# mbed92/soft-grip

Hardware: AMD Instinct MI355X
Metric: env steps/sec (whole node) at batch=4096 (higher is better)
Workload: dtype f64; 1 GPU; configs[2]: 4096 envs/GPU, softbox scene (nv=118), stiffness ~ U(300,1400), reference 200-step squeeze schedule from reset, 7 substeps per env step; 327 equality rows (composite neighbour equalities on: DESIGN.md 2, U2); volume tendon damper integrated explicitly; envs_per_gpu=4096, envs_flagged_bad=0

## Files before the change

### soft-grip_amd/csrc/sg_api.hip

```cpp
#include <cstdio>
#include <cstring>
#include <memory>

#include "sg_batch.h"
#include "sg_blob.h"
#include "sg_mjcf.h"
#include "sg_tree.h"
#ifdef SG_LEGACY_PIPELINES
#include "sg_kernels_args.h"
#define SG_LEGACY_ON 1
#else
#define SG_LEGACY_ON 0
#endif

static thread_local std::string g_err;
int fail(int code, const std::string& msg) {
  g_err = msg;
  return code;
}
int devmem_fail(bool nomem, const std::string& what) {
  (void)hipGetLastError();
  return fail(nomem ? SG_ERR_NOMEM : SG_ERR_HIP, what + (nomem ? ": out of device memory" : ": a HIP memset, copy or synchronise failed"));
}

namespace {
__global__ void sg_fill_rows_kernel(double* dst, const double* row, int n, int w) {
  int i = blockIdx.x * blockDim.x + threadIdx.x;
  if (i < n * w) dst[i] = row[i % w];
}
#define SG_CTRL_BYVAL 8
struct SgCtrlRow { double v[SG_CTRL_BYVAL]; };
__global__ void sg_fill_rows_val_kernel(double* dst, SgCtrlRow row, int n, int w) {
  int i = blockIdx.x * blockDim.x + threadIdx.x;
  if (i < n * w) dst[i] = row.v[i % w];
}
__global__ void sg_masked_copy_kernel(const unsigned char* mask, int n, const int* s0, int* d0, const int* s1, int* d1, const int* s2, int* d2,
                                      const int* s3, int* d3, const int* s4, int* d4) {
  int i = blockIdx.x * blockDim.x + threadIdx.x;
  if (i < n && (!mask || mask[i])) { d0[i] = s0[i]; d1[i] = s1[i]; d2[i] = s2[i]; d3[i] = s3[i]; d4[i] = s4[i]; }
}
}

static int begin_event_pair(sg_batch* b, std::vector<std::pair<hipEvent_t, hipEvent_t>>& list, hipStream_t s);

static int tree_alloc(sg_batch* b) {
  if (b->tree_ready) return SG_OK;
  const sg_model* m = b->m;
  if (!m->has_tree) return fail(SG_ERR_MODEL, "the tree pipeline does not run this model");
  const size_t n = b->n;
  SgArena& A = b->tree_mem;
  SgTreeBufs& t = b->t;
  bool ok = A.zeros(&t.H, 1) && A.zeros(&t.T, 1) && A.upload(&t.elem, m->tplan.elem) && A.upload(&t.pairs, m->tplan.gpairs) &&
            A.zeros(&t.cws, n * (size_t)m->tree_cws) && A.zeros(&t.touch_words, 2 * n) && A.upload(&t.sched, m->tplan.sched) &&
            A.upload(&t.nbtab, m->tplan.nbtab) && hipMemcpy(t.H, &m->tplan.h, sizeof(SgPlanHeader), hipMemcpyHostToDevice) == hipSuccess &&
            hipMemcpy(t.T, &m->tree, sizeof(SgTreeDev), hipMemcpyHostToDevice) == hipSuccess;
  if (!ok) {
    A.release();
    t = SgTreeBufs();
    return devmem_fail(A.nomem, "tree pipeline");
  }
  b->tree_ready = true;
  return SG_OK;
}

static int rows_alloc(sg_batch* b) {
  SgRowsBufs& r = b->r;
  if (r.ready) return SG_OK;
  const sg_model* m = b->m;
  const SgPlanHeader& H = m->plan.h;
  SgArena& A = b->rows_mem;
  r.shape = sg_rows_shape(H);
  r.nsl = sg_rows_nsl(H.nelem);
  r.w.secprof = b->secprof;
  bool ok = A.zeros(&r.H, 1) && hipMemcpy(r.H, &H, sizeof H, hipMemcpyHostToDevice) == hipSuccess && A.upload(&r.elem, m->plan.elem) &&
            A.upload(&r.gpairs, m->plan.gpairs) &&
            sg_rows_work_each(r.w, H, m->rounds, (size_t)b->n, SG_LEGACY_ON != 0, [&A](auto** p, size_t count) { return A.zeros(p, count); });
  if (ok && r.shape.nb_mode) {
    SgRowsTables T;
    sg_rows_tables(m->plan, &T);
    ok = A.upload(&r.nbtab, m->plan.nbtab) && A.upload(&r.sched, T.sched) && A.upload(&r.tab, T.tab) && A.upload(&r.cpos, T.cpos);
  }
  if (!ok) {
    A.release();
    r = SgRowsBufs();
    return devmem_fail(A.nomem, "rows pipeline");
  }
  r.ready = true;
  return SG_OK;
}

static int launch_tree(sg_batch* b, int mode, const uint8_t* mask, int nsub, double* sens, long long stride, int32_t* flags, int32_t* touch,
                       hipStream_t s) {
  const sg_model* m = b->m;
  sgt::TreeArgs a;
  a.H = b->t.H; a.T = b->t.T; a.elem = b->t.elem; a.gpairs = b->t.pairs; a.sched = b->t.sched; a.nbtab = b->t.nbtab;
  a.qpos = b->qpos; a.qvel = b->qvel; a.warm = b->warm; a.act = b->act; a.ctrl = b->ctrl;
  a.kenv = b->kenv; a.kmask_jnt = b->kmask_jnt; a.kmask_ten = b->kmask_ten;
  a.mask = mask; a.sens = sens; a.sens_stride = stride > 0 ? stride : m->tplan.h.nsensordata;
  a.flags = flags ? flags : b->flags; a.touch = touch ? touch : b->touch; a.touch_words = b->t.touch_words;
  a.ncon = b->ncon; a.nefc = b->nefc; a.iters = b->iters;
  a.cws = b->t.cws; a.cws_stride = m->tree_cws;
  a.nenv = b->n; a.nsub = nsub; a.mode = mode; a.secprof = b->secprof;
  if (!b->tree_attr_set) {
    HIPCHK(sg_tree_prepare());
    b->tree_attr_set = true;
  }
  if (b->prof)
    if (int rc = begin_event_pair(b, b->ev, s)) return rc;
  HIPCHK(sg_launch_tree(a, m->tree.CS, m->tree_lds, s));
  if (b->prof) HIPCHK(hipEventRecord(b->ev.back().second, s));
  return SG_OK;
}

extern "C" {

const char* sg_last_error(void) { return g_err.c_str(); }
const char* sg_version(void) { return "softgrip-mi355x 0.1 (gfx950)"; }

int sg_model_create(const void* blob, size_t nbytes, sg_model** out) {
  if (!blob || !out) return fail(SG_ERR_INVALID, "sg_model_create: null argument");
  sg_model* m = new sg_model();
  std::string err, terr;
  m->has_fast = sg_plan_build(blob, nbytes, &m->plan, &err);
  m->has_tree = sg_tree_plan_build(blob, nbytes, &m->tplan, &m->tree, &terr);
  if (m->has_tree) {
    m->tree_lds = sgt::lds_bytes(m->tree, m->tplan.h.nelem, m->tplan.h.has_free, m->tplan.h.nnb);
    m->tree_cws = sgt::cws_doubles(m->tree, m->tplan.h.nelem, m->tplan.h.has_free, m->tplan.h.nnb);
  }
  if (m->has_tree && m->tree_lds > 160 * 1024) {
    m->has_tree = false;
    terr = "the env's state does not fit the 160 KB of LDS";
  }
  if (!m->has_fast && !m->has_tree) {
    delete m;
    return fail(SG_ERR_MODEL, "sg_model_create: " + err + " (two-finger kernels); " + terr + " (tree pipeline)");
  }
  if (!m->has_fast) m->plan = m->tplan;
  sgk_build(blob, nbytes, m->has_fast ? m->plan : m->tplan, m->has_tree ? &m->tree : nullptr, m->has_fast, &m->kin);
  sgc_from_blob(blob, nbytes, m->kin, &m->con);
  m->rounds = (m->plan.h.nelem + 63) / 64;
  if (m->rounds > 4) {
    delete m;
    return fail(SG_ERR_MODEL, "sg_model_create: more than 256 composite elements");
  }
  if (m->has_fast && !sg_rows_admits(m->plan.h, &err)) {
    delete m;
    return fail(SG_ERR_MODEL, "sg_model_create: " + err);
  }
  *out = m;
  return SG_OK;
}
void sg_model_destroy(sg_model* m) { delete m; }

int sg_mjcf_compile(const char* xml_path, int flags, void** blob, size_t* nbytes) {
  if (!xml_path || !blob || !nbytes) return fail(SG_ERR_INVALID, "sg_mjcf_compile: null argument");
  std::string out, err;
  if (!sg_mjcf_compile_file(xml_path, !(flags & SG_COMPILE_NO_NEIGHBORS), (flags & SG_COMPILE_IMPLICIT_TENDON_DAMPER) != 0, &out, &err))
    return fail(SG_ERR_MODEL, "sg_mjcf_compile: " + err);
  void* p = malloc(out.size());
  if (!p) return fail(SG_ERR_INVALID, "sg_mjcf_compile: out of memory");
  memcpy(p, out.data(), out.size());
  *blob = p; *nbytes = out.size();
  return SG_OK;
}
void sg_blob_free(void* blob) { free(blob); }

int sg_model_compile(const char* xml_path, int flags, sg_model** out) {
  if (!xml_path || !out) return fail(SG_ERR_INVALID, "sg_model_compile: null argument");
  std::string blob, err;
  SgSkinSpec spec;
  if (!sg_mjcf_compile_file(xml_path, !(flags & SG_COMPILE_NO_NEIGHBORS), (flags & SG_COMPILE_IMPLICIT_TENDON_DAMPER) != 0, &blob, &err, &spec))
    return fail(SG_ERR_MODEL, "sg_mjcf_compile: " + err);
  int rc = sg_model_create(blob.data(), blob.size(), out);
  if (rc != SG_OK || !spec.present) return rc;
  long long c = 0;
  const char* names = (const char*)sg_blob_find(blob.data(), blob.size(), "names", SG_DT_U8, &c);
  std::vector<std::string> body_names(1);
  for (long long i = 0; names && i < c && names[i] != '\n'; i++) {
    if (names[i] == '|') body_names.emplace_back();
    else body_names.back().push_back(names[i]);
  }
  SgSkinHost S;
  if (sg_composite_skin(body_names, &spec.prefix, spec.inflate, spec.rgba, &S) &&
      sg_model_set_skin(*out, S.nvert, S.vert_body.data(), S.vert_pos.data(), S.nface, S.face.data(), S.rgba) != SG_OK)
    (void)sg_model_set_skin(*out, 0, nullptr, nullptr, 0, nullptr, nullptr);
  return SG_OK;
}
int sg_model_nq(const sg_model* m) { return m->plan.h.nq; }
int sg_model_nv(const sg_model* m) { return m->plan.h.nv; }
int sg_model_njnt(const sg_model* m) { return m->plan.h.njnt; }
int sg_model_nu(const sg_model* m) { return m->plan.h.nu; }
int sg_model_nsensordata(const sg_model* m) { return m->plan.h.nsensordata; }
int sg_model_ntendon(const sg_model* m) { return m->plan.h.ntendon; }
int sg_model_nelem(const sg_model* m) { return m->plan.h.nelem; }

void sg_batch_destroy(sg_batch* b) {
  if (!b) return;
  (void)hipSetDevice(b->device);
  delete b;
}

static int first_pipeline(const sg_model* m) {
  if (!m->has_fast) return 3;
  const char* pm = getenv("SG_PIPELINE");
  int p = (pm && strcmp(pm, "tree") == 0 && m->has_tree) ? 3 : 2;
#ifdef SG_LEGACY_PIPELINES
  if (pm && strcmp(pm, "fused") == 0) p = 0;
  if (pm && strcmp(pm, "split") == 0) p = 1;
#endif
  if (m->plan.h.nnb > 0 && p != 3) p = 2;
  return p;
}

int sg_batch_create(const sg_model* m, int n_envs, int device, sg_batch** out) {
  if (!m || !out || n_envs <= 0) return fail(SG_ERR_INVALID, "sg_batch_create: bad argument");
  int ndev = 0;
  if (hipGetDeviceCount(&ndev) != hipSuccess || ndev <= 0) return fail(SG_ERR_NO_DEVICE, "sg_batch_create: no HIP device (there is no CPU fallback)");
  if (device < 0 || device >= ndev) return fail(SG_ERR_NO_DEVICE, "sg_batch_create: device index out of range");
  HIPCHK(hipSetDevice(device));
  std::unique_ptr<sg_batch, void (*)(sg_batch*)> guard(new sg_batch(), sg_batch_destroy);
  sg_batch* b = guard.get();
  b->m = m; b->n = n_envs; b->device = device;
  SgArena& A = b->mem;
  const SgPlanHeader& H = m->plan.h;
  const size_t n = n_envs, nv = H.nv, nq = H.nq, njnt = H.njnt, nu = H.nu, nt = H.ntendon;
  bool ok = A.zeros(&b->qpos, n * nq) && A.zeros(&b->qvel, n * nv) && A.zeros(&b->warm, n * nv) && A.zeros(&b->act, n * nu) &&
            A.zeros(&b->ctrl, n * nu) && A.zeros(&b->kenv, n) && A.zeros(&b->ctrl_row, nu) && A.zeros(&b->kmask_jnt, njnt) &&
            A.zeros(&b->kmask_ten, nt) && A.zeros(&b->flags, n) && A.zeros(&b->touch, n) && A.zeros(&b->ncon, n) && A.zeros(&b->nefc, n) &&
            A.zeros(&b->iters, n) && A.zeros(&b->secprof, 48);
  if (!ok) return devmem_fail(A.nomem, "sg_batch_create (state)");
  b->kmask_jnt_host.assign(njnt, 0); b->kmask_ten_host.assign(nt, 0);
  b->pipeline = first_pipeline(m);
  if (int rc = b->pipeline == 3 ? tree_alloc(b) : rows_alloc(b)) return rc;
  std::vector<double> q0(nq, 0.0);
  for (int c = 0; c < H.nchain; c++)
    for (int d = 0; d < H.chain[c].ndof; d++) q0[H.chain[c].dof0 + d] = H.chain[c].qpos0[d];
  if (!m->has_fast)
    for (int d = 0; d < m->tree.ND; d++) q0[m->tree.d_gid[d]] = m->tree.d_qpos0[d];
  for (int e = 0; e < H.nelem; e++) q0[H.elem_qpos0 + e] = m->plan.elem[(size_t)SGE_QPOS0 * H.nelem + e];
  if (H.has_free)
    for (int c = 0; c < 7; c++) q0[H.free_qadr + c] = H.free_q0[c];
  std::vector<double> qall(n * nq);
  for (size_t i = 0; i < n; i++) memcpy(&qall[i * nq], q0.data(), sizeof(double) * nq);
  HIPCHK(hipMemcpy(b->qpos, qall.data(), sizeof(double) * n * nq, hipMemcpyHostToDevice));
  *out = guard.release();
  return SG_OK;
}
int sg_batch_nenvs(const sg_batch* b) { return b->n; }
int sg_batch_device(const sg_batch* b) { return b->device; }

int sg_set_stiffness(sg_batch* b, const double* k, int k_on_host, const int* jnt_ids, int nj, const int* ten_ids, int nt, void* stream) {
  if (!b || !k || nj < 0 || nt < 0 || (nj && !jnt_ids) || (nt && !ten_ids)) return fail(SG_ERR_INVALID, "sg_set_stiffness: bad argument");
  HIPCHK(hipSetDevice(b->device));
  const SgPlanHeader& H = b->m->plan.h;
  std::vector<int> mj(H.njnt, 0), mt(H.ntendon, 0);
  for (int i = 0; i < nj; i++) {
    if (jnt_ids[i] < 0 || jnt_ids[i] >= H.njnt) return fail(SG_ERR_INVALID, "sg_set_stiffness: joint id out of range");
    mj[jnt_ids[i]] = 1;
  }
  for (int i = 0; i < nt; i++) {
    if (ten_ids[i] < 0 || ten_ids[i] >= H.ntendon) return fail(SG_ERR_INVALID, "sg_set_stiffness: tendon id out of range");
    mt[ten_ids[i]] = 1;
  }
  hipStream_t s = (hipStream_t)stream;
  const bool masks_changed = mj != b->kmask_jnt_host || mt != b->kmask_ten_host;
  if (masks_changed || k_on_host) HIPCHK(hipStreamSynchronize(s));
  if (masks_changed) {
    HIPCHK(hipMemcpy(b->kmask_jnt, mj.data(), sizeof(int) * H.njnt, hipMemcpyHostToDevice));
    HIPCHK(hipMemcpy(b->kmask_ten, mt.data(), sizeof(int) * H.ntendon, hipMemcpyHostToDevice));
    b->kmask_jnt_host = mj;
    b->kmask_ten_host = mt;
  }
  if (k_on_host) HIPCHK(hipMemcpy(b->kenv, k, sizeof(double) * b->n, hipMemcpyHostToDevice));
  else HIPCHK(hipMemcpyAsync(b->kenv, k, sizeof(double) * b->n, hipMemcpyDeviceToDevice, s));
  return SG_OK;
}

int sg_set_ctrl(sg_batch* b, const double* ctrl, int broadcast, void* stream) {
  if (!b || !ctrl) return fail(SG_ERR_INVALID, "sg_set_ctrl: bad argument");
  HIPCHK(hipSetDevice(b->device));
  hipStream_t s = (hipStream_t)stream;
  const int nu = b->m->plan.h.nu;
  if (nu == 0) return SG_OK;
  if (broadcast && nu <= SG_CTRL_BYVAL) {
    SgCtrlRow row;
    for (int i = 0; i < SG_CTRL_BYVAL; i++) row.v[i] = i < nu ? ctrl[i] : 0.0;
    int total = b->n * nu;
    hipLaunchKernelGGL(sg_fill_rows_val_kernel, dim3((total + 255) / 256), dim3(256), 0, s, b->ctrl, row, b->n, nu);
    HIPCHK(hipGetLastError());
  } else if (broadcast) {
    HIPCHK(hipStreamSynchronize(s));
    HIPCHK(hipMemcpy(b->ctrl_row, ctrl, sizeof(double) * nu, hipMemcpyHostToDevice));
    int total = b->n * nu;
    hipLaunchKernelGGL(sg_fill_rows_kernel, dim3((total + 255) / 256), dim3(256), 0, s, b->ctrl, b->ctrl_row, b->n, nu);
    HIPCHK(hipGetLastError());
  } else {
    HIPCHK(hipMemcpyAsync(b->ctrl, ctrl, sizeof(double) * b->n * nu, hipMemcpyDeviceToDevice, s));
  }
  return SG_OK;
}

static int begin_event_pair(sg_batch* b, std::vector<std::pair<hipEvent_t, hipEvent_t>>& list, hipStream_t s) {
  hipEvent_t e[2];
  for (int i = 0; i < 2; i++) {
    if (!b->ev_pool.empty()) { e[i] = b->ev_pool.back(); b->ev_pool.pop_back(); }
    else if (hipEventCreate(&e[i]) != hipSuccess) {
      if (i == 1) b->ev_pool.push_back(e[0]);
      return fail(SG_ERR_HIP, "hipEventCreate failed");
    }
  }
  list.emplace_back(e[0], e[1]);
  HIPCHK(hipEventRecord(e[0], s));
  return SG_OK;
}

static int profile_read(sg_batch* b, std::vector<std::pair<hipEvent_t, hipEvent_t>>& list, double& sum_ms, long long& count, int reset, double* avg_ms,
                        long long* launches) {
  HIPCHK(hipSetDevice(b->device));
  for (auto& e : list) {
    HIPCHK(hipEventSynchronize(e.second));
    float ms = 0;
    HIPCHK(hipEventElapsedTime(&ms, e.first, e.second));
    sum_ms += ms; count++;
    b->ev_pool.push_back(e.first); b->ev_pool.push_back(e.second);
  }
  list.clear();
  if (avg_ms) *avg_ms = count ? sum_ms / count : 0.0;
  if (launches) *launches = count;
  if (reset) { sum_ms = 0; count = 0; }
  return SG_OK;
}

#define SG_EPW8_MIN_WAVES 1024
static int solver_epw(const sg_batch* b) {
  if (b->m->plan.h.nnb > 0) return 4;
  if (b->epw_override) return b->epw_override;
  if (const char* pe = getenv("SG_PGS_EPW")) return atoi(pe) == 4 ? 4 : 8;
  return (b->n + 7) / 8 >= SG_EPW8_MIN_WAVES ? 8 : 4;
}

static int launch_split(sg_batch* b, int mode, const uint8_t* mask, int nsub, double* sens, long long stride, int32_t* flags, int32_t* touch,
                        hipStream_t s) {
  const SgPlanHeader& H = b->m->plan.h;
  SgRowsBufs& r = b->r;
  SgPhaseArgs pa;
  pa.H = r.H; pa.elem = r.elem;
  pa.qpos = b->qpos; pa.qvel = b->qvel; pa.warm = b->warm; pa.act = b->act; pa.ctrl = b->ctrl;
  pa.kenv = b->kenv; pa.kmask_jnt = b->kmask_jnt; pa.kmask_ten = b->kmask_ten;
  pa.mask = mask; pa.sens = nullptr; pa.sens_stride = stride > 0 ? stride : H.nsensordata;
  pa.w = r.w; pa.nenv = b->n; pa.rowlayout = b->pipeline == 2;
  pa.nbtab = r.nbtab; pa.cpos = r.cpos; pa.cst_rounds = r.shape.cst_rounds;
  pa.gpairs = r.gpairs;
  pa.nelem = H.nelem; pa.nv = H.nv; pa.nu = H.nu; pa.elem_dof0 = H.elem_dof0; pa.nchain = H.nchain; pa.t0_id = H.t0_id; pa.timestep = H.timestep;
  SgPgsArgs ga;
  ga.sched = r.sched; ga.nbtab = r.nbtab; ga.tab = r.tab;
  ga.H = r.H; ga.elem = r.elem; ga.w = r.w; ga.nenv = b->n;
#ifdef SG_LEGACY_PIPELINES
  const size_t lds = sizeof(double) * ((size_t)(5 * 8 + 2) * H.nelem + 16 * 4 * SG_MAXLIM + 72);
#endif
  const bool nbm = r.shape.nb_mode != 0;
  const int epw = solver_epw(b);
  const size_t lds_rows = sizeof(double) * r.shape.lds_doubles(epw, r.nsl);
  if (!r.attr_set) {
    HIPCHK(sg_rows_prepare());
#ifdef SG_LEGACY_PIPELINES
    HIPCHK(sg_legacy_prepare());
#endif
    r.attr_set = true;
  }
  const int nfwd = nsub + (mode == 1 ? 1 : 0);
  size_t call_ev = 0;
  if (b->prof) {
    if (int rc = begin_event_pair(b, b->ev, s)) return rc;
    call_ev = b->ev.size() - 1;
  }
  const bool genpass = b->pipeline == 2;
  for (int k = 0; k <= nfwd; k++) {
    SgPhaseArgs p = pa;
    p.first = k == 0;
    p.do_reset = (mode == 1 && k == 0);
    p.do_finish = k > 0;
    p.finish_integrate = (mode == 1) ? (k > 1) : 1;
    p.do_begin = k < nfwd;
    p.sens = (k == nfwd) ? sens : nullptr;
    if (nfwd == 0) { p.do_begin = 0; p.do_finish = 0; }
    HIPCHK(sg_launch_chain(p, b->n, s));
    p.sens = nullptr;
    HIPCHK(sg_launch_phase(p, b->m->rounds, nbm, genpass, b->n, s));
    if (k < nfwd) {
      if (b->prof)
        if (int rc = begin_event_pair(b, b->ev_pgs, s)) return rc;
      if (b->pipeline == 2) HIPCHK(sg_launch_rows(ga, r.nsl, r.shape.nb_mode, epw, b->n, lds_rows, s));
#ifdef SG_LEGACY_PIPELINES
      else HIPCHK(sg_launch_pgs_split(ga, b->n, lds, s));
#endif
      if (b->prof) HIPCHK(hipEventRecord(b->ev_pgs.back().second, s));
    }
  }
  if (b->prof) HIPCHK(hipEventRecord(b->ev[call_ev].second, s));
  hipLaunchKernelGGL(sg_masked_copy_kernel, dim3((b->n + 255) / 256), dim3(256), 0, s, mask, b->n, r.w.status, flags ? flags : b->flags,
                     r.w.touch, touch ? touch : b->touch, r.w.ncon, b->ncon, r.w.nefc, b->nefc, r.w.iters, b->iters);
  HIPCHK(hipGetLastError());
  return SG_OK;
}

static int launch(sg_batch* b, int mode, const uint8_t* mask, int nsub, double* sens, long long stride, int32_t* flags, int32_t* touch,
                  hipStream_t s) {
  if (b->pipeline == 3) return launch_tree(b, mode, mask, nsub, sens, stride, flags, touch, s);
  if (b->pipeline >= 1) return launch_split(b, mode, mask, nsub, sens, stride, flags, touch, s);
#ifdef SG_LEGACY_PIPELINES
  const SgPlanHeader& H = b->m->plan.h;
  SgKArgs a;
  a.H = b->r.H; a.elem = b->r.elem;
  a.qpos = b->qpos; a.qvel = b->qvel; a.warm = b->warm; a.act = b->act; a.ctrl = b->ctrl;
  a.kenv = b->kenv; a.kmask_jnt = b->kmask_jnt; a.kmask_ten = b->kmask_ten;
  a.mask = mask;
  a.sens = sens; a.sens_stride = stride > 0 ? stride : H.nsensordata;
  a.flags = flags ? flags : b->flags; a.touch = touch ? touch : b->touch;
  a.ncon = b->ncon; a.nefc = b->nefc; a.iters = b->iters;
  a.nenv = b->n; a.nsub = nsub; a.mode = mode;
  if (b->prof)
    if (int rc = begin_event_pair(b, b->ev, s)) return rc;
  HIPCHK(sg_launch_fused(a, b->m->rounds, b->n, s));
  if (b->prof) HIPCHK(hipEventRecord(b->ev.back().second, s));
  return SG_OK;
#else
  return fail(SG_ERR_MODEL, "the fused pipeline is not part of this build (test builds only: build_native.py --legacy)");
#endif
}

int sg_reset(sg_batch* b, const uint8_t* mask, int sim_start, double* sens_out, int32_t* flags_out, int32_t* touch_out, void* stream) {
  if (!b || sim_start < 0) return fail(SG_ERR_INVALID, "sg_reset: bad argument");
  HIPCHK(hipSetDevice(b->device));
  return launch(b, 1, mask, sim_start, sens_out, 0, flags_out, touch_out, (hipStream_t)stream);
}

int sg_step(sg_batch* b, int n_substeps, double* sens_out, long long sens_stride, int32_t* flags_out, int32_t* touch_out, void* stream) {
  if (!b || n_substeps < 0) return fail(SG_ERR_INVALID, "sg_step: bad argument");
  HIPCHK(hipSetDevice(b->device));
  return launch(b, 0, nullptr, n_substeps, sens_out, sens_stride, flags_out, touch_out, (hipStream_t)stream);
}

int sg_get_state(sg_batch* b, double* qpos, double* qvel, double* act, double* warm, double* ctrl, void* stream) {
  if (!b) return fail(SG_ERR_INVALID, "sg_get_state: bad argument");
  HIPCHK(hipSetDevice(b->device));
  hipStream_t s = (hipStream_t)stream;
  const size_t n = b->n, nv = b->m->plan.h.nv, nu = b->m->plan.h.nu;
  if (qpos) HIPCHK(hipMemcpyAsync(qpos, b->qpos, sizeof(double) * n * b->m->plan.h.nq, hipMemcpyDeviceToDevice, s));
  if (qvel) HIPCHK(hipMemcpyAsync(qvel, b->qvel, sizeof(double) * n * nv, hipMemcpyDeviceToDevice, s));
  if (warm) HIPCHK(hipMemcpyAsync(warm, b->warm, sizeof(double) * n * nv, hipMemcpyDeviceToDevice, s));
  if (act && nu) HIPCHK(hipMemcpyAsync(act, b->act, sizeof(double) * n * nu, hipMemcpyDeviceToDevice, s));
  if (ctrl && nu) HIPCHK(hipMemcpyAsync(ctrl, b->ctrl, sizeof(double) * n * nu, hipMemcpyDeviceToDevice, s));
  return SG_OK;
}

int sg_set_state(sg_batch* b, const double* qpos, const double* qvel, const double* act, const double* warm, const double* ctrl, void* stream) {
  if (!b) return fail(SG_ERR_INVALID, "sg_set_state: bad argument");
  HIPCHK(hipSetDevice(b->device));
  hipStream_t s = (hipStream_t)stream;
  const size_t n = b->n, nv = b->m->plan.h.nv, nu = b->m->plan.h.nu;
  if (qpos) HIPCHK(hipMemcpyAsync(b->qpos, qpos, sizeof(double) * n * b->m->plan.h.nq, hipMemcpyDeviceToDevice, s));
  if (qvel) HIPCHK(hipMemcpyAsync(b->qvel, qvel, sizeof(double) * n * nv, hipMemcpyDeviceToDevice, s));
  if (warm) HIPCHK(hipMemcpyAsync(b->warm, warm, sizeof(double) * n * nv, hipMemcpyDeviceToDevice, s));
  if (act && nu) HIPCHK(hipMemcpyAsync(b->act, act, sizeof(double) * n * nu, hipMemcpyDeviceToDevice, s));
  if (ctrl && nu) HIPCHK(hipMemcpyAsync(b->ctrl, ctrl, sizeof(double) * n * nu, hipMemcpyDeviceToDevice, s));
  return SG_OK;
}

int sg_get_solver_stats(sg_batch* b, int32_t* ncon, int32_t* nefc, int32_t* iters, void* stream) {
  if (!b) return fail(SG_ERR_INVALID, "sg_get_solver_stats: bad argument");
  HIPCHK(hipSetDevice(b->device));
  hipStream_t s = (hipStream_t)stream;
  const size_t n = b->n;
  if (ncon) HIPCHK(hipMemcpyAsync(ncon, b->ncon, sizeof(int) * n, hipMemcpyDeviceToDevice, s));
  if (nefc) HIPCHK(hipMemcpyAsync(nefc, b->nefc, sizeof(int) * n, hipMemcpyDeviceToDevice, s));
  if (iters) HIPCHK(hipMemcpyAsync(iters, b->iters, sizeof(int) * n, hipMemcpyDeviceToDevice, s));
  return SG_OK;
}

int sg_set_pipeline(sg_batch* b, int pipeline) {
  if (!b || pipeline < 0 || pipeline > 3) return fail(SG_ERR_INVALID, "sg_set_pipeline: bad argument");
  if (pipeline == 3) {
    if (!b->m->has_tree) return fail(SG_ERR_MODEL, "sg_set_pipeline: the tree pipeline does not run this model (fix-rows-only models within its capacities)");
    HIPCHK(hipSetDevice(b->device));
    if (int rc = tree_alloc(b)) return rc;
    b->pipeline = 3;
    return SG_OK;
  }
  if (!b->m->has_fast) return fail(SG_ERR_MODEL, "sg_set_pipeline: the model is outside the two-finger class, only the tree pipeline runs it");
#ifndef SG_LEGACY_PIPELINES
  if (pipeline < 2) return fail(SG_ERR_MODEL, "sg_set_pipeline: the fused and split pipelines are not part of this build (test builds only: build_native.py --legacy)");
#endif
  if (b->m->plan.h.nnb > 0 && pipeline != 2)
    return fail(SG_ERR_MODEL, "sg_set_pipeline: the model has neighbour equality rows, which only the rows pipeline supports");
  HIPCHK(hipSetDevice(b->device));
  if (int rc = rows_alloc(b)) return rc;
  b->pipeline = pipeline;
  return SG_OK;
}

int sg_get_touch_words(sg_batch* b, int32_t* out, int nwords, void* stream) {
  if (!b || !out || nwords < 1) return fail(SG_ERR_INVALID, "sg_get_touch_words: bad argument");
  HIPCHK(hipSetDevice(b->device));
  hipStream_t s = (hipStream_t)stream;
  HIPCHK(hipMemsetAsync(out, 0, sizeof(int32_t) * (size_t)b->n * nwords, s));
  if (b->pipeline == 3)
    HIPCHK(hipMemcpy2DAsync(out, sizeof(int32_t) * nwords, b->t.touch_words, sizeof(int32_t) * 2, sizeof(int32_t) * (nwords < 2 ? nwords : 2), b->n,
                            hipMemcpyDeviceToDevice, s));
  else
    HIPCHK(hipMemcpy2DAsync(out, sizeof(int32_t) * nwords, b->pipeline == 0 ? b->touch : b->r.w.touch, sizeof(int32_t), sizeof(int32_t), b->n,
                            hipMemcpyDeviceToDevice, s));
  return SG_OK;
}
int sg_model_nboxes(const sg_model* m) {
  if (!m) return 0;
  if (!m->has_fast) return m->tree.NG;
  int n = 0;
  for (int c = 0; c < m->plan.h.nchain; c++) n += m->plan.h.chain[c].ngeom;
  return n;
}

int sg_set_solver_envs_per_wavefront(sg_batch* b, int epw) {
  if (!b || (epw != 0 && epw != 4 && epw != 8)) return fail(SG_ERR_INVALID, "sg_set_solver_envs_per_wavefront: 0 (automatic), 4 or 8");
  if (b->m->plan.h.nnb > 0 && epw == 8)
    return fail(SG_ERR_MODEL, "sg_set_solver_envs_per_wavefront: a model with neighbour equality rows runs 4 envs of 16 lanes per wavefront");
  b->epw_override = epw;
  return SG_OK;
}
int sg_solver_envs_per_wavefront(const sg_batch* b) { return b ? solver_epw(b) : 0; }
int sg_tree_workgroups_per_cu(const sg_batch* b) {
  if (!b) return fail(SG_ERR_INVALID, "sg_tree_workgroups_per_cu: bad argument");
  if (!b->tree_ready) return 0;
  const sg_model* m = b->m;
  if (hipSetDevice(b->device) != hipSuccess) return fail(SG_ERR_NO_DEVICE, "hipSetDevice");
  if (sg_tree_prepare() != hipSuccess) return fail(SG_ERR_HIP, "sg_tree_prepare");
  return sg_tree_occupancy(m->tree.CS, m->tree_lds);
}

#ifdef SG_SECTION_PROF
int sg_debug_sections(sg_batch* b, unsigned long long* out32) {
  if (!b || !out32) return fail(SG_ERR_INVALID, "sg_debug_sections: bad argument");
  HIPCHK(hipSetDevice(b->device));
  HIPCHK(hipDeviceSynchronize());
  HIPCHK(hipMemcpy(out32, b->secprof, sizeof(unsigned long long) * 48, hipMemcpyDeviceToHost));
  HIPCHK(hipMemset(b->secprof, 0, sizeof(unsigned long long) * 48));
  return SG_OK;
}
#endif

#ifdef SG_DEBUG_WORK
long long sg_debug_tree_work(sg_batch* b, int env, double* out, long long cap) {
  if (!b || !out || env < 0 || env >= b->n || !b->t.cws) return fail(SG_ERR_INVALID, "sg_debug_tree_work: bad argument");
  const sg_model* m = b->m;
  long long n = m->tree_cws;
  if (n > cap) n = cap;
  HIPCHK(hipSetDevice(b->device));
  HIPCHK(hipDeviceSynchronize());
  HIPCHK(hipMemcpy(out, b->t.cws + (size_t)env * m->tree_cws, sizeof(double) * n, hipMemcpyDeviceToHost));
  return n;
}
#endif

int sg_profile_enable(sg_batch* b, int enable) {
  if (!b) return fail(SG_ERR_INVALID, "sg_profile_enable: bad argument");
  b->prof = enable != 0;
  return SG_OK;
}

int sg_profile_read_solver(sg_batch* b, int reset, double* avg_ms, long long* launches) {
  if (!b) return fail(SG_ERR_INVALID, "sg_profile_read_solver: bad argument");
  return profile_read(b, b->ev_pgs, b->prof_pgs_ms, b->prof_pgs_n, reset, avg_ms, launches);
}

int sg_profile_read(sg_batch* b, int reset, double* avg_ms, long long* launches) {
  if (!b) return fail(SG_ERR_INVALID, "sg_profile_read: bad argument");
  return profile_read(b, b->ev, b->prof_ms, b->prof_n, reset, avg_ms, launches);
}

int sg_model_nbody(const sg_model* m) { return m ? m->kin.o.nbody : 0; }
int sg_model_ngeom(const sg_model* m) { return m ? m->kin.o.ngeom : 0; }

}
```

### soft-grip_amd/csrc/sg_phase.hip

```cpp
#include "sg_work.h"

struct GenLds {
  StageRec2* stage;
  double* gas;
  double* gg;
  double* tmp;
  const double (*boxp)[3];
  const double (*boxm)[9];
  const ChainKin* K;
  const ChainLds2* cs;
  const double *qe, *ve, *asme, *we;
};

__device__ __forceinline__ void sg_gen_capsule(const SgPhaseArgs& a, const GenLds& L, int e, double* cp, double* cax) {
  const int N = a.nelem;
  auto EL = [&](int f, int k) { return a.elem[(size_t)f * N + k]; };
  const double dq = L.qe[e] - EL(SGE_QPOS0, e);
  cp[0] = EL(SGE_GX, e) + EL(SGE_AX, e) * dq; cp[1] = EL(SGE_GY, e) + EL(SGE_AY, e) * dq; cp[2] = EL(SGE_GZ, e) + EL(SGE_AZ, e) * dq;
  cax[0] = EL(SGE_CX, e); cax[1] = EL(SGE_CY, e); cax[2] = EL(SGE_CZ, e);
}

__device__ __noinline__ int sg_gen_phase(const SgPhaseArgs& a, const SgPlanHeader& H, const int env, const GenLds L, int* flags, int* touch) {
  const int lane = threadIdx.x, N = a.nelem;
  auto EL = [&](int f, int k) { return a.elem[(size_t)f * N + k]; };
  const SgWork& W = a.w;
  int ng = 0, fl = 0;
#pragma unroll 1
  for (int p0 = 0; p0 < H.ngpair; p0 += 64) {
    const int pi = p0 + lane;
    const bool have = pi < H.ngpair;
    SgGenPair gp;
    gp.kind = SGP_UNSUPPORTED; gp.g1 = gp.g2 = 0; gp.pad = 0;
    if (have) gp = a.gpairs[pi];
    ConRec r0, r1;
    int n = 0;
    bool big = false;
    if (have) {
      double cp[3] = {0, 0, 0}, cax[3] = {0, 0, 1};
      if (gp.kind == SGP_PLANE_CAP) {
        sg_gen_capsule(a, L, sgg_index(gp.g2), cp, cax);
        const double dif[3] = {cp[0] - H.plane_pos[0], cp[1] - H.plane_pos[1], cp[2] - H.plane_pos[2]};
        if (!(dot3(dif, H.plane_normal) > H.con_margin + H.cap_rbound))
          n = gen_plane_capsule(H.plane_pos, H.plane_normal, cp, cax, H.cap_radius, H.cap_hl, H.con_margin, r0, r1);
      } else if (gp.kind == SGP_PLANE_BOX) {
        const double *p2, *R2, *s2;
        double rb2;
        gen_box_of(gp.g2, H, L.boxp, L.boxm, p2, R2, s2, rb2);
        const double dif[3] = {p2[0] - H.plane_pos[0], p2[1] - H.plane_pos[1], p2[2] - H.plane_pos[2]};
        big = !(dot3(dif, H.plane_normal) > H.con_margin + rb2);
      } else {
        const double *p1 = nullptr, *R1 = nullptr, *s1 = nullptr, *p2, *R2, *s2;
        double rb1 = 0, rb2;
        const bool boxes = sgg_kind(gp.g1) == SGG_BOX || sgg_kind(gp.g1) == SGG_STATIC;
        if (gp.kind == SGP_SPH_BOX) { cp[0] = H.center_pos[0]; cp[1] = H.center_pos[1]; cp[2] = H.center_pos[2]; rb1 = H.center_radius; }
        else if (gp.kind == SGP_CAP_BOX) { sg_gen_capsule(a, L, sgg_index(gp.g1), cp, cax); rb1 = H.cap_rbound; }
        else if (boxes) { gen_box_of(gp.g1, H, L.boxp, L.boxm, p1, R1, s1, rb1); cp[0] = p1[0]; cp[1] = p1[1]; cp[2] = p1[2]; }
        if (gp.kind == SGP_UNSUPPORTED && !boxes) fl |= SG_FLAG_UNSUPPORTED_PAIR;
        else {
          gen_box_of(gp.g2, H, L.boxp, L.boxm, p2, R2, s2, rb2);
          const double dif[3] = {p2[0] - cp[0], p2[1] - cp[1], p2[2] - cp[2]}, bound = rb1 + rb2 + H.con_margin;
          if (dot3(dif, dif) <= bound * bound) {
            if (gp.kind == SGP_SPH_BOX) n = sphere_box(cp, H.center_radius, p2, R2, s2, H.con_margin, r0);
            else if (gp.kind == SGP_CAP_BOX) {
              const int mk = capsule_box(cp, cax, H.cap_radius, H.cap_hl, p2, R2, s2, H.con_margin, r0, r1);
              if ((mk & 2) && !(mk & 1)) r0 = r1;
              n = (mk & 1) + ((mk >> 1) & 1);
            } else big = true;
          }
        }
      }
      if (n == 2 && !(r1.dist < H.con_margin)) n = 1;
      if (n >= 1 && !(r0.dist < H.con_margin)) { r0 = r1; n--; }
    }
    unsigned long long todo = __ballot(n > 0 || big);
#pragma unroll 1
    while (todo) {
      const unsigned long long bigm = __ballot(big) & todo;
      const int Lb = bigm ? __ffsll((long long)bigm) - 1 : 64;
      const unsigned long long seg = Lb == 64 ? todo : (todo & ((1ull << Lb) - 1ull));
      const bool mine = (seg >> lane) & 1ull;
      const unsigned long long m1 = __ballot(mine && n >= 1), m2 = __ballot(mine && n >= 2);
      const int base = ng + lanes_below2(m1) + lanes_below2(m2);
      auto put = [&](int at, const ConRec& r) {
        StageRec2& o = L.stage[at];
        o.dist = r.dist; o.sl = pi; o.box = 0;
        for (int q = 0; q < 3; q++) { o.pos[q] = r.pos[q]; o.n[q] = r.n[q]; }
      };
      if (mine && n >= 1 && base < SG_GEN_MAXCON) put(base, r0);
      if (mine && n >= 2 && base + 1 < SG_GEN_MAXCON) put(base + 1, r1);
      ng += __popcll(m1) + __popcll(m2);
      todo &= ~seg;
      if (Lb < 64) {
        const int pb = p0 + Lb;
        const SgGenPair gb = a.gpairs[pb];
        int cnt = 0;
        if (lane == 0) {
          const int room = SG_GEN_MAXCON - (ng < SG_GEN_MAXCON ? ng : SG_GEN_MAXCON);
          StageRec2* out = L.stage + (ng < SG_GEN_MAXCON ? ng : 0);
          const double *p2, *R2, *s2;
          double rb2;
          gen_box_of(gb.g2, H, L.boxp, L.boxm, p2, R2, s2, rb2);
          int nb = 0;
          if (room >= 8) {
            if (gb.kind == SGP_PLANE_BOX) nb = gen_plane_box(H.plane_pos, H.plane_normal, p2, R2, s2, H.con_margin, out);
            else {
              const double *p1, *R1, *s1;
              double rb1;
              gen_box_of(gb.g1, H, L.boxp, L.boxm, p1, R1, s1, rb1);
              nb = gen_box_box(p1, R1, s1, p2, R2, s2, H.con_margin, out, (double (*)[3])L.tmp, (double (*)[3])(L.tmp + 48));
            }
            for (int q = 0; q < nb; q++)
              if (out[q].dist < H.con_margin) { if (cnt != q) out[cnt] = out[q]; out[cnt].sl = pb; cnt++; }
            if (gb.kind == SGP_UNSUPPORTED && cnt > 0) { cnt = 0; fl |= SG_FLAG_UNSUPPORTED_PAIR; }
          } else {
            fl |= SG_FLAG_CONTACTFULL;
          }
        }
        ng += __shfl(cnt, 0);
        todo &= ~(1ull << Lb);
        if (lane == Lb) big = false;
      }
    }
  }
  if (ng > SG_GEN_MAXCON) { ng = SG_GEN_MAXCON; fl |= SG_FLAG_CONTACTFULL; }
  __syncthreads();
  double Minv2[SG_MAXCH][16], vc2[SG_MAXCH][SG_CD], asm2[SG_MAXCH][SG_CD], warm2[SG_MAXCH][SG_CD];
#pragma unroll
  for (int c = 0; c < SG_MAXCH; c++) {
#pragma unroll
    for (int i = 0; i < 16; i++) Minv2[c][i] = L.cs[c].Minv[i];
#pragma unroll
    for (int d = 0; d < SG_CD; d++) { vc2[c][d] = L.cs[c].v[d]; asm2[c][d] = L.cs[c].qacc_smooth[d]; warm2[c][d] = L.cs[c].w[d]; }
  }
  double gsum[SG_MAXCH][SG_CD] = {{0, 0, 0, 0}, {0, 0, 0, 0}}, push[SG_GEN_ROUNDS];
  int slk[SG_GEN_ROUNDS], tch = 0;
  StageRec2 rec[SG_GEN_ROUNDS];
#pragma unroll
  for (int k = 0; k < SG_GEN_ROUNDS; k++)
    if (lane + 64 * k < ng) rec[k] = L.stage[lane + 64 * k];
  __syncthreads();
#pragma unroll
  for (int k = 0; k < SG_GEN_ROUNDS; k++) {
    const int i = lane + 64 * k;
    push[k] = 0; slk[k] = -1;
    if (i < ng) {
      const SgGenPair gp = a.gpairs[rec[k].sl];
      const GenSide S1 = gen_side_of(gp.g1, H, a.elem + (size_t)SGE_BINVW * N), S2 = gen_side_of(gp.g2, H, a.elem + (size_t)SGE_BINVW * N);
      const int sl = S1.sl >= 0 ? S1.sl : S2.sl;
      double ax[3] = {0, 0, 0}, hint[3] = {0, 0, 0}, ve_ = 0, as_ = 0, we_ = 0, im = 0;
      if (sl >= 0) {
        ax[0] = EL(SGE_AX, sl); ax[1] = EL(SGE_AY, sl); ax[2] = EL(SGE_AZ, sl);
        ve_ = L.ve[sl]; as_ = L.asme[sl]; we_ = L.we[sl];
        im = 1.0 / (EL(SGE_MASS, sl) + EL(SGE_ARMATURE, sl));
      }
      if (gp.kind == SGP_PLANE_CAP) { hint[0] = EL(SGE_CX, sl); hint[1] = EL(SGE_CY, sl); hint[2] = EL(SGE_CZ, sl); }
      GenContact c;
      gen_contact_build(c, rec[k], gp.kind == SGP_PLANE_CAP ? hint : nullptr, S1, S2, L.K, Minv2, vc2, asm2, warm2, ax, ve_, as_, we_, im, H);
      gen_contact_store(W.gcon + ((size_t)env * SG_GEN_MAXCON + i) * SG_GEN_W, c);
#pragma unroll
      for (int ch = 0; ch < SG_MAXCH; ch++)
#pragma unroll
        for (int d = 0; d < SG_CD; d++) gsum[ch][d] += c.Jf[ch][0][d] * c.f[0] + c.Jf[ch][1][d] * c.f[1] + c.Jf[ch][2][d] * c.f[2];
      slk[k] = sl;
      push[k] = c.invm * (c.Js[0] * c.f[0] + c.Js[1] * c.f[1] + c.Js[2] * c.f[2]);
      if ((gp.kind == SGP_CAP_BOX || gp.kind == SGP_SPH_BOX) && sgg_kind(gp.g2) == SGG_BOX) tch |= 1 << sgg_index(gp.g2);
    }
  }
  double* const gpush = (double*)L.stage;
  int* const gsl = (int*)(gpush + SG_GEN_MAXCON);
#pragma unroll
  for (int k = 0; k < SG_GEN_ROUNDS; k++)
    if (lane + 64 * k < SG_GEN_MAXCON) { gpush[lane + 64 * k] = push[k]; gsl[lane + 64 * k] = slk[k]; }
#pragma unroll
  for (int ch = 0; ch < SG_MAXCH; ch++)
#pragma unroll
    for (int d = 0; d < SG_CD; d++) {
      const double x = wave_sum2(gsum[ch][d]);
      if (lane == 0) L.gg[ch * SG_CD + d] = x;
    }
  __syncthreads();
  for (int e = lane; e < N; e += 64) {
    double acc = 0;
    for (int i = 0; i < ng; i++)
      if (gsl[i] == e) acc += gpush[i];
    L.gas[e] = acc;
  }
  int t = 0;
#pragma unroll
  for (int bb = 0; bb < SG_MAXCH * SG_CG; bb++)
    if (__ballot((tch >> bb) & 1)) t |= 1 << bb;
  *touch = t;
  int f2 = 0;
#pragma unroll
  for (int bit = 0; bit < 6; bit++)
    if (__ballot((fl >> bit) & 1)) f2 |= 1 << bit;
  *flags = f2;
  __syncthreads();
  return ng;
}

__device__ __noinline__ double sg_gen_cost(const SgPhaseArgs& a, const int env, const int ng, const double (*aF)[SG_CD], const double* as_lds,
                                           const int zero) {
  const int lane = threadIdx.x;
  double cp = 0;
  for (int i = lane; i < ng; i += 64) {
    double* rec = a.w.gcon + ((size_t)env * SG_GEN_MAXCON + i) * SG_GEN_W;
    if (zero) { rec[SG_GEN_F_OFF] = rec[SG_GEN_F_OFF + 1] = rec[SG_GEN_F_OFF + 2] = 0.0; continue; }
    GenContact c;
    gen_contact_load(c, rec);
    const double as_ = c.sl >= 0 ? as_lds[c.sl] : 0.0;
#pragma unroll
    for (int r = 0; r < 3; r++) {
      double Ja = c.Js[r] * as_;
#pragma unroll
      for (int ch = 0; ch < SG_MAXCH; ch++)
#pragma unroll
        for (int d = 0; d < SG_CD; d++) Ja += c.Jf[ch][r][d] * aF[ch][d];
      cp += c.f[r] * (0.5 * (Ja + c.R * c.f[r]) + c.b[r]);
    }
  }
  return cp;
}

template <int R, int CPL, bool NB, bool GEN>
__device__ __forceinline__ void sg_phase_env(const SgPhaseArgs& a, const int env) {
  const int lane = threadIdx.x;
  if (env >= a.nenv) return;
  if (a.mask && !a.mask[env]) return;
  SG_T0();
  const SG_CONSTAS SgPlanHeader& H = *(const SG_CONSTAS SgPlanHeader*)a.H;
  const int N = a.nelem, nv = a.nv, nu = a.nu, e0 = a.elem_dof0, nchain = a.nchain;
  const size_t S = 2 * (size_t)a.nenv;
  const double h = a.timestep;
  __shared__ Smem2<R, CPL, NB> Sm;
  const SG_CONSTAS double* const elemc = (const SG_CONSTAS double*)a.elem;
  [[maybe_unused]] const SG_CONSTAS int* const nbtabc = (const SG_CONSTAS int*)a.nbtab;
  auto EL = [&](int f, int e) { return elemc[(size_t)f * N + e]; };
  const int half = lane >> 5;
  const bool high = half != 0;
  const bool is_chain_lane = (lane & 31) == 0 && half < nchain;
  const SG_CONSTAS SgChain& C = H.chain[half < nchain ? half : 0];
  ChainLds2& CS = Sm.cs[half];
  const SgWork& W = a.w;
  [[maybe_unused]] unsigned short* const gpairs_env = W.gpairs16 + (size_t)env * SG_PAIRS_CAP(R);
  [[maybe_unused]] double* const gcval_env = W.gcval + (size_t)env * SG_MAXCH * (32 * CPL);
  auto pair_at = [&](int i) -> unsigned short& {
    if constexpr (SG_PHASE_SLIM(R)) return gpairs_env[i];
    else return Sm.pairs[i];
  };
  auto cval_at = [&](int cc, int i) -> double& {
    if constexpr (SG_PHASE_SLIM(R)) return gcval_env[cc * (32 * CPL) + i];
    else return Sm.cval[cc * (32 * CPL) + i];
  };

  int status = W.status[env];
  const int pend = W.pending[env];

  double* gq = a.qpos + (size_t)env * nv;
  double* gv = a.qvel + (size_t)env * nv;
  double* gw = a.warm + (size_t)env * nv;
  const double kenv = a.kenv[env];
  const int kt0_masked = a.kmask_ten[a.t0_id];

  double qe[R], ve[R], we[R], ke[R];
#pragma unroll
  for (int r = 0; r < R; r++) {
    int e = r * 64 + lane;
    qe[r] = ve[r] = we[r] = ke[r] = 0;
    if (e < N) {
      if (a.do_reset) { qe[r] = EL(SGE_QPOS0, e); }
      else { qe[r] = gq[e0 + e]; ve[r] = gv[e0 + e]; we[r] = gw[e0 + e]; }
      ke[r] = a.kmask_jnt[e0 + e] ? kenv : EL(SGE_K0, e);
    }
  }
  double ase[R], asme_p[R], fsm_p[R];
#pragma unroll
  for (int r = 0; r < R; r++) {
    const int e = r * 64 + lane;
    ase[r] = asme_p[r] = fsm_p[r] = 0;
    if (a.do_finish && e < N) {
      ase[r] = W.as[(size_t)env * N + e]; asme_p[r] = W.asme[(size_t)env * N + e];
      if (a.finish_integrate) fsm_p[r] = W.fsm[(size_t)env * N + e];
    }
  }
  if (a.do_begin && half < nchain) {
    const double* ch = W.chh + ((size_t)env * 2 + half) * SG_CHW;
    double* const kd = (double*)&Sm.K[half];
    double* const box = &Sm.boxp[half * SG_CG][0];
    double* const boxm = &Sm.boxm[half * SG_CG][0];
    double* const lim = CS.lim_sign;
#pragma unroll
    for (int j0 = 0; j0 < SG_CHW; j0 += 32) {
      const int j = j0 + (lane & 31);
      const double v = j < SG_CHW ? ch[j] : 0.0;
      if (j >= SGH_QSM && j < SGH_QSM + SG_CD) CS.qacc_smooth[j - SGH_QSM] = v;
      else if (j >= SGH_K && j < SGH_K + SGH_N_K) kd[j - SGH_K] = v;
      else if (j >= SGH_MINV && j < SGH_MINV + SGH_N_M) CS.Minv[j - SGH_MINV] = v;
      else if (j >= SGH_V && j < SGH_V + SG_CD) CS.v[j - SGH_V] = v;
      else if (j >= SGH_W && j < SGH_W + SG_CD) CS.w[j - SGH_W] = v;
      else if (j >= SGH_BOX && j < SGH_BOX + SGH_N_BOX) {
        const int g = (j - SGH_BOX) / SGH_N_BOX1, k = (j - SGH_BOX) % SGH_N_BOX1;
        if (k < 3) box[3 * g + k] = v; else boxm[9 * g + k - 3] = v;
      }
      else if (j == SGH_LIMACT) CS.lim_active = (int)v;
      else if (j >= SGH_LIMSIGN && j < SGH_LIMSIGN + SGH_N_LIM) lim[j - SGH_LIMSIGN] = v;
    }
  }
  const bool dead = (status & (SG_FLAG_BADQPOS | SG_FLAG_BADQVEL | SG_FLAG_BADQACC)) != 0;
  if (dead) return;
  const bool fin = a.do_finish && pend;
  const double kt0 = kt0_masked ? kenv : H.t0_k0;
  __syncthreads();

  SG_T(0);
  if (fin) {
    int badacc = 0;
    double qacc_e[R];
#pragma unroll
    for (int r = 0; r < R; r++) {
      int e = r * 64 + lane;
      qacc_e[r] = 0;
      if (e < N) {
        qacc_e[r] = asme_p[r] + ase[r];
        if (isbad(qacc_e[r])) badacc = 1;
      }
    }
    const bool anybadacc = __ballot(badacc) != 0;
    if (anybadacc) {
      status |= SG_FLAG_BADQACC;
    } else {
      double qa[R], yc[R];
      double Sp = 0;
#pragma unroll
      for (int r = 0; r < R; r++) {
        int e = r * 64 + lane;
        we[r] = qacc_e[r];
        qa[r] = yc[r] = 0;
        if (e < N && a.finish_integrate) {
          double m = EL(SGE_MASS, e) + EL(SGE_ARMATURE, e);
          double den = m + h * EL(SGE_DAMPING, e);
          qa[r] = (fsm_p[r] + m * ase[r]) / den;
          if (H.t0_implicit) { const double cf = EL(SGE_COEF, e); yc[r] = cf / den; Sp += cf * qa[r]; }
        }
      }
      if (H.t0_implicit && a.finish_integrate) {
        const double kk = h * H.t0_damping * wave_sum2(Sp) / (1.0 + H.t0_hcT);
#pragma unroll
        for (int r = 0; r < R; r++) qa[r] -= yc[r] * kk;
      }
#pragma unroll
      for (int r = 0; r < R; r++) {
        int e = r * 64 + lane;
        if (e < N && a.finish_integrate) {
          ve[r] += h * qa[r];
          qe[r] += h * ve[r];
        }
      }
    }
    if (lane == 0) W.pending[env] = 0;
  }
  __syncthreads();

  SG_T(1);
  int flags = 0;
  if (a.do_begin && !(status & SG_FLAG_BADQACC)) {
    int bad = 0;
#pragma unroll
    for (int r = 0; r < R; r++) bad |= (isbad(qe[r]) ? SG_FLAG_BADQPOS : 0) | (isbad(ve[r]) ? SG_FLAG_BADQVEL : 0);
    if (__ballot(bad != 0)) {
      flags |= (__ballot(bad & 1) ? 1 : 0) | (__ballot(bad & 2) ? 2 : 0);
    } else {
      double invm[R], asme[R], coef[R];
      double L0p = 0, Ldp = 0;
#pragma unroll
      for (int r = 0; r < R; r++) {
        int e = r * 64 + lane;
        coef[r] = e < N ? EL(SGE_COEF, e) : 0.0;
        L0p += coef[r] * qe[r]; Ldp += coef[r] * ve[r];
      }
      const double L0 = wave_sum2(L0p), Ld = wave_sum2(Ldp);
      const double frc_t0 = -kt0 * (L0 - H.t0_lspring) - H.t0_damping * Ld;
      int unsupported = 0, ns0 = 0, ns1 = 0, touch = 0;
      bool special = false;
      {
        double cpos[R][3];
#pragma unroll
        for (int r = 0; r < R; r++) {
          int e = r * 64 + lane;
          invm[r] = asme[r] = 0;
          cpos[r][0] = cpos[r][1] = cpos[r][2] = 1e30;
          if (e < N) {
            double ax[3] = {EL(SGE_AX, e), EL(SGE_AY, e), EL(SGE_AZ, e)}, m = EL(SGE_MASS, e);
            double bias = -m * dot3(H.gravity, ax);
            double f = -ke[r] * (qe[r] - EL(SGE_SPRINGREF, e)) - EL(SGE_DAMPING, e) * ve[r] + coef[r] * frc_t0 - bias;
            invm[r] = 1.0 / (m + EL(SGE_ARMATURE, e));
            asme[r] = f * invm[r];
            W.fsm[(size_t)env * N + e] = f; W.asme[(size_t)env * N + e] = asme[r];
            double dq = qe[r] - EL(SGE_QPOS0, e);
            cpos[r][0] = EL(SGE_GX, e) + ax[0] * dq; cpos[r][1] = EL(SGE_GY, e) + ax[1] * dq; cpos[r][2] = EL(SGE_GZ, e) + ax[2] * dq;
            if (!(qe[r] > EL(SGE_QLO, e) && qe[r] < EL(SGE_QHI, e))) unsupported = 1;
            Sm.ve[e] = ve[r]; Sm.asme[e] = asme[r]; Sm.we[e] = we[r];
            *(unsigned int*)&Sm.eslot[e][0] = 0u;
            Sm.as[e] = qe[r];
          }
        }
        SG_T(2);
        __syncthreads();
        int overflow = 0;
        int np = 0;
#pragma unroll 1
        for (int b = 0; b < nchain * SG_CG; b++) {
          const int c = b / SG_CG, g = b % SG_CG;
          const SgChain& Cc = H.chain[c];
          if (g >= Cc.ngeom) continue;
          double bp[3], bm[9], sz[3];
#pragma unroll
          for (int k = 0; k < 3; k++) { bp[k] = Sm.boxp[b][k]; sz[k] = Cc.g_size[g][k]; }
#pragma unroll
          for (int k = 0; k < 9; k++) bm[k] = Sm.boxm[b][k];
          const double rb = Cc.g_rbound[g];
          if (H.has_center) {
            double dif[3] = {bp[0] - H.center_pos[0], bp[1] - H.center_pos[1], bp[2] - H.center_pos[2]}, bound = H.center_radius + rb + H.con_margin;
            if (dot3(dif, dif) <= bound * bound) {
              if (lane == 0) pair_at(np) = (unsigned short)((b << 12) | SG_PAIR_CENTER);
              np++;
            }
          }
#pragma unroll
          for (int r = 0; r < R; r++) {
            const int e = r * 64 + lane;
            double dif[3] = {cpos[r][0] - bp[0], cpos[r][1] - bp[1], cpos[r][2] - bp[2]}, bound = H.cap_rbound + rb + H.con_margin;
            bool near = e < N && dot3(dif, dif) <= bound * bound;
            if (near) {
              double lc[3], grow = H.cap_rbound + H.con_margin;
              mulmatT3(lc, bm, dif);
              near = fabs(lc[0]) <= sz[0] + grow && fabs(lc[1]) <= sz[1] + grow && fabs(lc[2]) <= sz[2] + grow;
              if (near) {
                const double cax[3] = {EL(SGE_CX, e), EL(SGE_CY, e), EL(SGE_CZ, e)}, rm = H.cap_radius + H.con_margin;
                double hb[3];
                mulmatT3(hb, bm, cax);
                near = fabs(lc[0]) <= sz[0] + rm + H.cap_hl * fabs(hb[0]) && fabs(lc[1]) <= sz[1] + rm + H.cap_hl * fabs(hb[1]) &&
                       fabs(lc[2]) <= sz[2] + rm + H.cap_hl * fabs(hb[2]);
              }
            }
            const unsigned long long m = __ballot(near);
            if (near) pair_at(np + lanes_below2(m)) = (unsigned short)((b << 12) | e);
            np += __popcll(m);
          }
        }
        __syncthreads();
        int nsc[SG_MAXCH] = {0, 0};
#pragma unroll 1
        for (int p0 = 0; p0 < np; p0 += 64) {
          const bool have = p0 + lane < np;
          const int code = have ? (int)pair_at(p0 + lane) : 0, b = code >> 12, e = code & 0xFFF, c = b / SG_CG, g = b % SG_CG;
          const bool is_center = have && e == SG_PAIR_CENTER;
          ConRec r0, r1;
          bool v0 = false, v1 = false;
          double bp[3], bm[9], sz[3];
#pragma unroll
          for (int k = 0; k < 3; k++) { bp[k] = Sm.boxp[b][k]; sz[k] = H.chain[c].g_size[g][k]; }
#pragma unroll
          for (int k = 0; k < 9; k++) bm[k] = Sm.boxm[b][k];
          if (__ballot(is_center)) {
            if (is_center) v0 = sphere_box(H.center_pos, H.center_radius, bp, bm, sz, H.con_margin, r0) && r0.dist < H.con_margin;
          }
          if (have && !is_center) {
            const double dq = Sm.as[e] - EL(SGE_QPOS0, e);
            double cp[3] = {EL(SGE_GX, e) + EL(SGE_AX, e) * dq, EL(SGE_GY, e) + EL(SGE_AY, e) * dq, EL(SGE_GZ, e) + EL(SGE_AZ, e) * dq};
            double cax[3] = {EL(SGE_CX, e), EL(SGE_CY, e), EL(SGE_CZ, e)};
            int mk = capsule_box(cp, cax, H.cap_radius, H.cap_hl, bp, bm, sz, H.con_margin, r0, r1);
            v0 = (mk & 1) && r0.dist < H.con_margin;
            v1 = (mk & 2) && r1.dist < H.con_margin;
          }
          const int n = (int)v0 + (int)v1;
#pragma unroll
          for (int cc = 0; cc < SG_MAXCH; cc++) {
            const bool mine = have && c == cc;
            const unsigned long long m1 = __ballot(mine && n >= 1), m2 = __ballot(mine && n >= 2);
            const int base = nsc[cc] + lanes_below2(m1) + lanes_below2(m2);
            if (mine && v0 && base < 32 * CPL) {
              StageRec2& s = Sm.stage[cc][base];
              s.dist = r0.dist; s.sl = is_center ? -1 : e; s.box = g;
              for (int q = 0; q < 3; q++) { s.pos[q] = r0.pos[q]; s.n[q] = r0.n[q]; }
            }
            if (mine && v1 && base + (int)v0 < 32 * CPL) {
              StageRec2& s = Sm.stage[cc][base + (int)v0];
              s.dist = r1.dist; s.sl = e; s.box = g;
              for (int q = 0; q < 3; q++) { s.pos[q] = r1.pos[q]; s.n[q] = r1.n[q]; }
            }
            if (mine && n > 0 && !is_center) {
              const int room = 32 * CPL - base, nst = n < room ? n : (room > 0 ? room : 0);
              static_assert(32 * CPL <= 64, "a contact slot index must fit 6 bits");
              Sm.eslot[e][b] = nst ? (unsigned char)(base | (nst << 6)) : (unsigned char)0;
            }
            nsc[cc] += __popcll(m1) + __popcll(m2);
            if (nsc[cc] > 32 * CPL) { nsc[cc] = 32 * CPL; overflow = 1; }
          }
#pragma unroll
          for (int bb = 0; bb < SG_MAXCH * SG_CG; bb++)
            if (__ballot(n > 0 && b == bb)) touch |= 1 << bb;
        }
        ns0 = nsc[0]; ns1 = nsc[1];
#ifdef SG_SECTION_PROF
        if (lane == 0) { atomicAdd(&a.w.secprof[30], (unsigned long long)np); atomicAdd(&a.w.secprof[31], (unsigned long long)((np + 63) / 64)); }
#endif
        if (overflow) flags |= SG_FLAG_CONTACTFULL;
      }
      SG_T(3);
      {
        int nb = nchain * SG_CG, npairs = nb * H.nstatic;
        const double *p1 = nullptr, *R1 = nullptr, *s1 = nullptr, *p2 = nullptr, *R2 = nullptr, *s2 = nullptr;
        double bd = 0;
        bool pair = false;
        if (lane < npairs) {
          int b = lane / H.nstatic, s = lane % H.nstatic, c = b / SG_CG, g = b % SG_CG;
          if (g < H.chain[c].ngeom) {
            pair = true;
            p1 = Sm.boxp[b]; R1 = Sm.boxm[b]; s1 = H.chain[c].g_size[g];
            p2 = H.st_pos[s]; R2 = H.st_mat[s]; s2 = H.st_size[s];
            bd = H.chain[c].g_rbound[g] + H.st_rbound[s];
          }
        } else if (lane >= 32 && lane < 32 + SG_CG * SG_CG && nchain == 2) {
          int g = (lane - 32) / SG_CG, g2 = (lane - 32) % SG_CG;
          if (g < H.chain[0].ngeom && g2 < H.chain[1].ngeom) {
            int b = g, b2 = SG_CG + g2;
            pair = true;
            p1 = Sm.boxp[b]; R1 = Sm.boxm[b]; s1 = H.chain[0].g_size[g];
            p2 = Sm.boxp[b2]; R2 = Sm.boxm[b2]; s2 = H.chain[1].g_size[g2];
            bd = H.chain[0].g_rbound[g] + H.chain[1].g_rbound[g2];
          }
        }
        if (pair) {
          double dif[3] = {p1[0] - p2[0], p1[1] - p2[1], p1[2] - p2[2]};
          if (dot3(dif, dif) <= bd * bd && box_box_overlap(p1, R1, s1, p2, R2, s2, 0)) unsupported = 1;
        }
        if (lane >= 48 && lane < 48 + SG_MAXCH * SG_CG && H.has_plane) {
          int b = lane - 48, c = b / SG_CG, g = b % SG_CG;
          if (c < nchain && g < H.chain[c].ngeom) {
            double dif[3] = {Sm.boxp[b][0] - H.plane_pos[0], Sm.boxp[b][1] - H.plane_pos[1], Sm.boxp[b][2] - H.plane_pos[2]}, ext = 0;
            for (int k = 0; k < 3; k++)
              ext += H.chain[c].g_size[g][k] * fabs(H.plane_normal[0] * Sm.boxm[b][k] + H.plane_normal[1] * Sm.boxm[b][3 + k] + H.plane_normal[2] * Sm.boxm[b][6 + k]);
            if (dot3(dif, H.plane_normal) - ext <= 0) unsupported = 1;
          }
        }
        special = __ballot(unsupported) != 0;
      }
      SG_T(4);
      __syncthreads();
      int ngen = 0;
      [[maybe_unused]] GenLds GL;
      if (special) {
        if (!a.rowlayout) flags |= SG_FLAG_UNSUPPORTED_PAIR;
        else if constexpr (!GEN) {
          if (lane == 0) a.w.gen_list[atomicAdd(a.w.gen_count, 1)] = env;
        } else {
          static_assert(sizeof(StageRec2) == 64 && sizeof(Sm.stage) >= 8 * (8 * SG_GEN_MAXCON + 96 + SG_MAXCH * SG_CD) &&
                        8 * SG_GEN_MAXCON >= SG_GEN_MAXCON + SG_GEN_MAXCON / 2 + R * 64, "the general path's lists live in the contact staging area");
          GL.stage = &Sm.stage[0][0];
          GL.gas = (double*)&Sm.stage[0][0] + SG_GEN_MAXCON + SG_GEN_MAXCON / 2;
          GL.tmp = (double*)&Sm.stage[0][0] + 8 * SG_GEN_MAXCON; GL.gg = GL.tmp + 96;
          GL.boxp = Sm.boxp; GL.boxm = Sm.boxm; GL.K = Sm.K; GL.cs = Sm.cs;
          GL.qe = Sm.as; GL.ve = Sm.ve; GL.asme = Sm.asme; GL.we = Sm.we;
          int gfl = 0, gtouch = 0;
          ngen = sg_gen_phase(a, *a.H, env, GL, &gfl, &gtouch);
          flags |= gfl;
          touch = gtouch;
          ns0 = ns1 = 0;
#pragma unroll
          for (int r = 0; r < R; r++) {
            const int e = r * 64 + lane;
            if (e < N) *(unsigned int*)&Sm.eslot[e][0] = 0u;
          }
          __syncthreads();
        }
      }
      int shared_slider = 0;
#pragma unroll
      for (int r = 0; r < R; r++) {
        int e = r * 64 + lane;
        static_assert(SG_MAXCH == 2 && SG_CG == 2, "the shared-slider test reads an element's four slot bytes as two halves");
        if (e < N && ((const unsigned short*)&Sm.eslot[e][0])[0] != 0 && ((const unsigned short*)&Sm.eslot[e][0])[1] != 0) shared_slider = 1;
      }
      shared_slider = __ballot(shared_slider) != 0;

      const int myn = high ? ns1 : ns0;
      const size_t st = SG_STREAM(env, half);
      const int nwb = (a.nenv + SG_EPW - 1) / SG_EPW;
      double cg[CPL][SG_CD], cjsf[CPL], cinvm[CPL], ccost0[CPL];
      int csl_[CPL];
#pragma unroll
      for (int k = 0; k < CPL; k++) {
        int i = (lane & 31) + 32 * k;
        csl_[k] = -1; cjsf[k] = cinvm[k] = ccost0[k] = 0;
#pragma unroll
        for (int d = 0; d < SG_CD; d++) cg[k][d] = 0;
        double2 fp[4][SG_RK / 2];
#pragma unroll
        for (int r = 0; r < 4; r++)
#pragma unroll
          for (int pr = 0; pr < SG_RK / 2; pr++) fp[r][pr] = make_double2(0.0, 0.0);
        if (i < myn) {
          Contact c;
          const StageRec2& sr = Sm.stage[half][i];
          ConRec rec;
          rec.dist = sr.dist;
          for (int q = 0; q < 3; q++) { rec.pos[q] = sr.pos[q]; rec.n[q] = sr.n[q]; }
          int sl = sr.sl, g = sr.box, bi = C.g_body[g], nd = chain_ndof_of_body(bi);
          double ax[3] = {0, 0, 0}, ve_ = 0, as_ = 0, we_ = 0, im = 0, bw = 0;
          if (sl >= 0) {
            ax[0] = EL(SGE_AX, sl); ax[1] = EL(SGE_AY, sl); ax[2] = EL(SGE_AZ, sl);
            ve_ = Sm.ve[sl]; as_ = Sm.asme[sl]; we_ = Sm.we[sl];
            im = 1.0 / (EL(SGE_MASS, sl) + EL(SGE_ARMATURE, sl)); bw = EL(SGE_BINVW, sl);
          }
          contact_build(c, rec, Sm.K[half], nd, CS.Minv, CS.v, CS.qacc_smooth, CS.w, C.b_invw_tran[bi], sl, ax, ve_, as_, we_, im, bw, *a.H);
          csl_[k] = sl; cinvm[k] = c.invm;
          cjsf[k] = c.Js[0] * c.f[0] + c.Js[1] * c.f[1] + c.Js[2] * c.f[2];
          cval_at(half, i) = c.invm * cjsf[k];
          ccost0[k] = c.f[0] * (0.5 * c.R * c.f[0] + c.b[0]) + c.f[1] * (0.5 * c.R * c.f[1] + c.b[1]) + c.f[2] * (0.5 * c.R * c.f[2] + c.b[2]);
#pragma unroll
          for (int d = 0; d < SG_CD; d++) cg[k][d] = c.Jf[0][d] * c.f[0] + c.Jf[1][d] * c.f[1] + c.Jf[2][d] * c.f[2];
          SG_T(24);
          if (a.rowlayout) {
            const double S11 = c.A[3] * H.con_mu[0] * H.con_mu[0], S22 = c.A[5] * H.con_mu[1] * H.con_mu[1], S12 = c.A[4] * H.con_mu[0] * H.con_mu[1];
            const double det = S11 * S22 - S12 * S12, di = det < 1e-10 ? 0.0 : sg_div(1.0, det);
            const double P11 = S22 * di, P22 = S11 * di, P12 = -S12 * di;
            double ecs = 1.0, esn = 0.0, ee1 = S11, ee2 = S22;
            if (fabs(S12) > 1e-300) {
              const double tau = (S22 - S11) / (2.0 * S12), tt = (tau >= 0 ? 1.0 : -1.0) / (fabs(tau) + sqrt(1.0 + tau * tau));
              ecs = 1.0 / sqrt(1.0 + tt * tt); esn = tt * ecs;
              ee1 = S11 - tt * S12; ee2 = S22 + tt * S12;
            }
            const double Afull[3][3] = {{c.A[0], c.A[1], c.A[2]}, {c.A[1], c.A[3], c.A[4]}, {c.A[2], c.A[4], c.A[5]}};
            double Wm[3][SG_CD];
#pragma unroll
            for (int r = 0; r < 3; r++)
#pragma unroll
              for (int d = 0; d < SG_CD; d++) {
                double sw = 0;
#pragma unroll
                for (int e = 0; e < SG_CD; e++) sw += c.Jf[r][e] * CS.Minv[4 * e + d];
                Wm[r][d] = sw;
              }
#pragma unroll
            for (int r = 0; r < 4; r++) {
              double fld[SG_RK];
#pragma unroll
              for (int q = 0; q < SG_RK; q++) fld[q] = 0.0;
              if (r < 3) {
#pragma unroll
                for (int d = 0; d < SG_CD; d++) fld[SGR_JF0 + d] = c.Jf[r][d];
                fld[SGR_JS] = c.Js[r]; fld[SGR_B] = c.b[r]; fld[SGR_F] = c.f[r];
                fld[SGR_AF] = Afull[r][0] * c.f[0] + Afull[r][1] * c.f[1] + Afull[r][2] * c.f[2];
                fld[SGR_A0] = Afull[r][0]; fld[SGR_A1] = Afull[r][1]; fld[SGR_A2] = Afull[r][2];
                fld[SGR_IMJS] = c.invm * c.Js[r];
                fld[SGR_R] = c.R;
              } else {
                fld[SGQ_P11] = P11; fld[SGQ_P12] = P12; fld[SGQ_P22] = P22; fld[SGQ_SLIDER] = __hiloint2double(0, sl);
                fld[SGQ_E1] = ee1; fld[SGQ_E2] = ee2; fld[SGQ_COS] = ecs; fld[SGQ_SIN] = esn;
              }
              fld[SGR_W0] = Wm[0][r]; fld[SGR_W1] = Wm[1][r]; fld[SGR_W2] = Wm[2][r];
#pragma unroll
              for (int pr = 0; pr < SG_RK / 2; pr++) fp[r][pr] = make_double2(fld[2 * pr], fld[2 * pr + 1]);
            }
          }
          if (!a.rowlayout) {
          double* ro = W.crec + SG_REC_INDEX(i, env / SG_EPW, 0, 2 * (env % SG_EPW) + half, nwb);
#pragma unroll
          for (int r = 0; r < 3; r++)
#pragma unroll
            for (int d = 0; d < SG_CD; d++) ro[(4 * r + d) * SG_SPW] = c.Jf[r][d];
#pragma unroll
          for (int r = 0; r < 3; r++) ro[(12 + r) * SG_SPW] = c.Js[r];
#pragma unroll
          for (int q = 0; q < 6; q++) ro[(15 + q) * SG_SPW] = c.A[q];
#pragma unroll
          for (int r = 0; r < 3; r++) ro[(21 + r) * SG_SPW] = c.b[r];
          ro[24 * SG_SPW] = c.R;
          ro[25 * SG_SPW] = c.invm;
#pragma unroll
          for (int r = 0; r < 3; r++) ro[(26 + r) * SG_SPW] = c.f[r];
          ((int*)(ro + 29 * SG_SPW))[0] = sl;
          }
        }
        const int nk = (ns0 > ns1 ? ns0 : ns1) - 32 * k;
        if (a.rowlayout && nk > 0) {
          const int nwb8 = (a.nenv + 7) / 8;
          const int li = lane & 31;
          auto X = [&](int sl_, int L) -> double2* {
            return (double2*)&Sm.stage[sl_ >> 4][32 * k] + ((sl_ & 15) * 8 + L);
          };
          __syncthreads();
          double2* const e0 = (double2*)&Sm.stage[li >> 4][32 * k] + ((li & 15) * 8 + 4 * half);
#pragma unroll
          for (int pr = 0; pr < SG_RK / 2; pr++) {
            e0[0] = fp[0][pr]; e0[1] = fp[1][pr]; e0[2] = fp[2][pr]; e0[3] = fp[3][pr];
            __syncthreads();
#pragma unroll
            for (int j = 0; j < 4; j++) {
              if (8 * j >= nk) break;
              const int e = j * 64 + lane, s_ = e >> 3, L = e & 7;
              if (s_ < nk) *(double2*)(W.crow + SG_ROW_INDEX(32 * k + s_, env >> 3, 2 * pr, 8 * (env & 7) + L, nwb8)) = *X(s_, L);
            }
            __syncthreads();
          }
        }
      }
      SG_T(5);
      double eqR[R], eqb[R], eqf[R];
      double tbp = 0, tjp = 0, tAp = 0;
#pragma unroll
      for (int r = 0; r < R; r++) {
        int e = r * 64 + lane;
        eqR[r] = 1; eqb[r] = 0; eqf[r] = 0;
        if (e < N) {
          double pos = qe[r] - EL(SGE_QPOS0, e), imp = impedance(H.eqj_solimp, pos, 0);
          eqR[r] = fmax(SG_MINVAL, (1 - imp) / imp * EL(SGE_INVW, e));
          double aref = -H.eqj_B * ve[r] - H.eqj_K * imp * pos;
          eqb[r] = asme[r] - aref;
          eqf[r] = -(we[r] - aref) / eqR[r];
          tbp += coef[r] * asme[r]; tjp += coef[r] * we[r]; tAp += coef[r] * coef[r] * invm[r];
        }
      }
      const int nnb = NB ? H.nnb : 0;
      constexpr int ND = NB ? 3 : 0;
      int nbe2[R][3], nbid[R][3];
      double nbc0[R][3];
      [[maybe_unused]] double nbff[R][3];
      [[maybe_unused]] double nbbb[R][3];
      [[maybe_unused]] double* const gnbf = W.nbf + (size_t)env * 3 * N;
#pragma unroll
      for (int r = 0; r < R; r++)
#pragma unroll
        for (int d = 0; d < 3; d++) { nbe2[r][d] = -1; nbid[r][d] = -1; nbc0[r][d] = 0; nbff[r][d] = 0; nbbb[r][d] = 0; }
      if constexpr (NB) {
        const double im0 = 1.0 / (EL(SGE_MASS, 0) + EL(SGE_ARMATURE, 0));
        const SG_CONSTAS int* const cposc = (const SG_CONSTAS int*)a.cpos;
        const bool ready = a.rowlayout != 0, wantc = ready && a.cst_rounds;
#pragma unroll
        for (int r = 0; r < R; r++) {
          const int e = r * 64 + lane;
          if (e < N) {
            double c4[4] = {0.0, 0.0, 0.0, 0.0}, g3[3] = {0.0, 0.0, 0.0};
            if (ready) c4[0] = sg_div(im0, im0 + eqR[r]);
#pragma unroll
            for (int d = 0; d < 3; d++) {
              const int e2 = nbtabc[d * N + e];
              if (e2 >= 0) {
                const int id = nbtabc[(3 + d) * N + e];
                const double pos = (qe[r] - EL(SGE_QPOS0, e)) - (Sm.as[e2] - EL(SGE_QPOS0, e2)), imp = impedance(H.eqj_solimp, pos, 0);
                const double Rr = fmax(SG_MINVAL, (1 - imp) / imp * (EL(SGE_INVW, e) + EL(SGE_INVW, e2)));
                const double aref = -H.eqj_B * (ve[r] - Sm.ve[e2]) - H.eqj_K * imp * pos;
                const double bb = (asme[r] - Sm.asme[e2]) - aref, ff = -((we[r] - Sm.we[e2]) - aref) / Rr;
                nbe2[r][d] = e2; nbid[r][d] = id; nbc0[r][d] = ff * (0.5 * Rr * ff + bb);
                nbff[r][d] = ff; gnbf[id] = ff;
                nbbb[r][d] = bb;
                if (ready) { g3[d] = fma(Rr, ff, bb); c4[1 + d] = sg_div(im0, 2.0 * im0 + Rr); }
                else { W.nbb[(size_t)env * 3 * N + id] = bb; W.nbR[(size_t)env * 3 * N + id] = Rr; }
              }
            }
            if (ready) {
              const size_t o3 = sg_eq_nb_index((size_t)env, e, 0, N);
#pragma unroll
              for (int d = 0; d < 3; d++) W.nbb[o3 + d] = g3[d];
              if (!wantc) {
                W.eqR[sg_eq_fix_index((size_t)env, e, N)] = c4[0];
#pragma unroll
                for (int d = 0; d < 3; d++) W.nbR[o3 + d] = c4[1 + d];
              }
            }
            if (wantc) {
              double* const dst = W.cst + SG_CST_INDEX(env >> 2, 0, 16 * (env & 3), a.cst_rounds) + cposc[e];
              *(double2*)dst = make_double2(c4[0], c4[1]);
              *(double2*)(dst + 2) = make_double2(c4[2], c4[3]);
            }
          }
        }
      }
      const double tpos = L0 - H.t0_L0, timp = impedance(H.eqt_solimp, tpos, 0), tR = fmax(SG_MINVAL, (1 - timp) / timp * H.eqt_invw);
      const double taref = -H.eqt_B * Ld - H.eqt_K * timp * tpos;
      const double tb = wave_sum2(tbp) - taref, tjar = wave_sum2(tjp) - taref, tA = wave_sum2(tAp) + tR;
      double tf = -tjar / tR;
      const int nmaxs = ns0 > ns1 ? ns0 : ns1;

      double aF[SG_CD];
      auto recompute_a = [&]() {
        __syncthreads();
#pragma unroll
        for (int r = 0; r < R; r++) {
          int e = r * 64 + lane;
          if (e < N) {
            double fe = eqf[r] + coef[r] * tf;
            if constexpr (NB) {
#pragma unroll
              for (int d = 0; d < 3; d++) if (nbid[r][d] >= 0) fe += nbff[r][d];
              double fin[3];
#pragma unroll
              for (int d = 0; d < 3; d++) { const int ii = nbtabc[(6 + d) * N + e]; fin[d] = ii >= 0 ? gnbf[ii] : 0.0; }
#pragma unroll
              for (int d = 0; d < 3; d++) fe -= fin[d];
            }
            double as_ = invm[r] * fe;
#pragma unroll
            for (int cb = 0; cb < SG_MAXCH * SG_CG; cb++) {
              const int u = Sm.eslot[e][cb], i0 = u & 0x3F, nst = u >> 6;
              if (nst >= 1) as_ += cval_at(cb / SG_CG, i0);
              if (nst >= 2) as_ += cval_at(cb / SG_CG, i0 + 1);
            }
            if constexpr (GEN)
              if (ngen) as_ += GL.gas[e];
            Sm.as[e] = as_;
          }
        }
        __syncthreads();
        double g[SG_CD] = {0, 0, 0, 0};
#pragma unroll
        for (int k = 0; k < CPL; k++)
#pragma unroll
          for (int d = 0; d < SG_CD; d++) g[d] += cg[k][d];
        if (is_chain_lane) {
          const int la = CS.lim_active;
#pragma unroll
          for (int k = 0; k < SG_MAXLIM; k++)
            if (la >> k & 1) g[k / 2] += CS.lim_sign[k] * CS.lim_f[k];
          if constexpr (GEN)
            if (ngen) {
#pragma unroll
              for (int d = 0; d < SG_CD; d++) g[d] += GL.gg[half * SG_CD + d];
            }
        }
#pragma unroll
        for (int d = 0; d < SG_CD; d++) {
          double x = g[d];
#pragma unroll
          for (int o = 16; o > 0; o >>= 1) x += __shfl_xor(x, o);
          g[d] = x;
        }
#pragma unroll
        for (int a2 = 0; a2 < SG_CD; a2++) {
          double s2 = 0;
#pragma unroll
          for (int b2 = 0; b2 < SG_CD; b2++) s2 += CS.Minv[4 * a2 + b2] * g[b2];
          aF[a2] = s2;
        }
        __syncthreads();
      };
      recompute_a();
      SG_T(6);
      {
        double cp = 0, tJap = 0;
#pragma unroll
        for (int r = 0; r < R; r++) {
          int e = r * 64 + lane;
          if (e < N) {
            double ae = Sm.as[e]; cp += eqf[r] * (0.5 * (ae + eqR[r] * eqf[r]) + eqb[r]); tJap += coef[r] * ae;
#pragma unroll
            for (int d = 0; d < ND; d++)
              if (nbid[r][d] >= 0) cp += 0.5 * nbff[r][d] * (ae - Sm.as[nbe2[r][d]]) + nbc0[r][d];
          }
        }
        double tJa = wave_sum2(tJap);
        if (lane == 0) cp += tf * (0.5 * (tJa + tR * tf) + tb);
        if (is_chain_lane) {
          const int la = CS.lim_active;
#pragma unroll
          for (int k = 0; k < SG_MAXLIM; k++)
            if (la >> k & 1) cp += CS.lim_f[k] * (0.5 * (CS.lim_sign[k] * aF[k / 2] + CS.lim_R[k] * CS.lim_f[k]) + CS.lim_b[k]);
        }
#pragma unroll
        for (int k = 0; k < CPL; k++)
          if ((lane & 31) + 32 * k < myn) {
            double as_ = csl_[k] >= 0 ? Sm.as[csl_[k]] : 0.0, ga = 0;
#pragma unroll
            for (int d = 0; d < SG_CD; d++) ga += cg[k][d] * aF[d];
            cp += 0.5 * (ga + cjsf[k] * as_) + ccost0[k];
          }
        [[maybe_unused]] double aF2[SG_MAXCH][SG_CD];
        if constexpr (GEN)
          if (ngen) {
#pragma unroll
            for (int d = 0; d < SG_CD; d++) {
              const double other = __shfl_xor(aF[d], 32);
              aF2[0][d] = high ? other : aF[d]; aF2[1][d] = high ? aF[d] : other;
            }
            cp += sg_gen_cost(a, env, ngen, aF2, Sm.as, 0);
          }
        double cost = wave_sum2(cp);
        if (cost > 0) {
          if constexpr (GEN)
            if (ngen) {
              sg_gen_cost(a, env, ngen, aF2, Sm.as, 1);
              for (int e = lane; e < N; e += 64) GL.gas[e] = 0.0;
              if (lane < SG_MAXCH * SG_CD) GL.gg[lane] = 0.0;
            }
#pragma unroll
          for (int r = 0; r < R; r++) {
            eqf[r] = 0;
#pragma unroll
            for (int d = 0; d < ND; d++)
              if (nbid[r][d] >= 0) {
                nbff[r][d] = 0.0; gnbf[nbid[r][d]] = 0.0;
                if (a.rowlayout) W.nbb[sg_eq_nb_index((size_t)env, r * 64 + lane, d, N)] = nbbb[r][d];
              }
          }
          tf = 0;
          if (is_chain_lane) {
#pragma unroll
            for (int k = 0; k < SG_MAXLIM; k++) CS.lim_f[k] = 0;
          }
#pragma unroll
          for (int k = 0; k < CPL; k++) {
            int i = (lane & 31) + 32 * k;
            cjsf[k] = 0;
#pragma unroll
            for (int d = 0; d < SG_CD; d++) cg[k][d] = 0;
            if (i < myn) {
              cval_at(half, i) = 0.0;
              if (!a.rowlayout) {
              double* ro = W.crec + SG_REC_INDEX(i, env / SG_EPW, 0, 2 * (env % SG_EPW) + half, nwb);
#pragma unroll
              for (int r = 0; r < 3; r++) ro[(26 + r) * SG_SPW] = 0.0;
              }
              if (a.rowlayout) {
#pragma unroll
                for (int r = 0; r < 3; r++)
                  *(double2*)(W.crow + SG_ROW_INDEX(i, env >> 3, SGR_F, 8 * (env & 7) + 4 * half + r, (a.nenv + 7) / 8)) = make_double2(0.0, 0.0);
              }
            }
          }
          __syncthreads();
          recompute_a();
        }
      }
      SG_T(7);
#pragma unroll
      for (int r = 0; r < R; r++) {
        int e = r * 64 + lane;
        if (e < N) {
          size_t o = (size_t)env * N + e;
          W.as[o] = Sm.as[e];
          if (NB && a.rowlayout) W.eqb[o] = fma(eqR[r], eqf[r], eqb[r]);
          else { W.eqf[o] = eqf[r]; W.eqb[o] = eqb[r]; W.eqR[o] = eqR[r]; }
        }
      }
      if (is_chain_lane) {
        W.ns[st] = myn < SG_CAP ? myn : SG_CAP;
        W.lim_active[st] = CS.lim_active;
      }
      if (half < nchain) {
        static_assert(SGH_N_LIM == 32, "one limit value per lane of a half");
        const int i = lane & 31;
        W.lim[SG_LIM_FLAT_INDEX(i, st, S)] = (&CS.lim_sign[0])[i];
        if (i < SG_CD) W.saF[SG_SAF_INDEX(i, st, S)] = i == 0 ? aF[0] : (i == 1 ? aF[1] : (i == 2 ? aF[2] : aF[3]));
      }
      if (lane == 0) {
        W.envh[SG_ENVH_INDEX(SG_ENVH_TB, env, a.nenv)] = tb; W.envh[SG_ENVH_INDEX(SG_ENVH_TR, env, a.nenv)] = tR;
        W.envh[SG_ENVH_INDEX(SG_ENVH_TA, env, a.nenv)] = tA; W.envh[SG_ENVH_INDEX(SG_ENVH_TF, env, a.nenv)] = tf;
        W.shared[env] = shared_slider;
        W.pending[env] = 1;
        W.ncon[env] = ns0 + ns1 + ngen;
        W.gen[env] = ngen;
        W.nefc[env] = N + nnb + 1 + 3 * (ns0 + ns1 + ngen) + __popc(Sm.cs[0].lim_active) + (nchain > 1 ? __popc(Sm.cs[1].lim_active) : 0);
        W.touch[env] = touch;
      }
    }
  }

  SG_T(8);
  __syncthreads();
#pragma unroll
  for (int r = 0; r < R; r++) {
    int e = r * 64 + lane;
    if (e < N) { gq[e0 + e] = qe[r]; gv[e0 + e] = ve[r]; gw[e0 + e] = we[r]; }
  }
  if (lane == 0) {
    if (status | flags) atomicOr(&W.status[env], status | flags);
  }
  SG_T(9);
  SG_TEND();
}

#ifndef SG_X_PHASE_OCC
#define SG_X_PHASE_OCC 2
#endif
#ifndef SG_X_CPL
#define SG_X_CPL 2
#endif
template <int R, int CPL, bool NB, bool GEN = false>
__global__ __launch_bounds__(64, SG_X_PHASE_OCC) void sg_phase_kernel(SgPhaseArgs a) {
  if constexpr (GEN) {
    const int cnt = a.w.gen_count[0];
    a.do_finish = 0; a.do_reset = 0; a.sens = nullptr;
    for (int i = blockIdx.x; i < cnt && i < a.nenv; i += gridDim.x) {
      sg_phase_env<R, CPL, NB, true>(a, a.w.gen_list[i]);
      __syncthreads();
    }
  } else {
    sg_phase_env<R, CPL, NB, false>(a, blockIdx.x);
  }
}

__global__ __launch_bounds__(64) void sg_chain_kernel(SgPhaseArgs a) {
  const int lane = threadIdx.x, c = blockIdx.x & 1, env = (int)(blockIdx.x >> 1) * 64 + lane;
  if (blockIdx.x == 0 && lane == 0) a.w.gen_count[0] = 0;
  SG_T0();
  const SG_CONSTAS SgPlanHeader& H = *(const SG_CONSTAS SgPlanHeader*)a.H;
  const int nv = a.nv, nu = a.nu;
  const size_t S = 2 * (size_t)a.nenv;
  if (env >= a.nenv) return;
  const size_t st = SG_STREAM(env, c);
  if (a.mask && !a.mask[env]) return;
  SgWork& W = a.w;
  if (a.first && c == 0) { W.status[env] = 0; if (!a.do_finish) W.pending[env] = 0; }
  if (c >= a.nchain) return;
  const int status = a.first ? 0 : W.status[env];
  const int pend = a.do_finish ? W.pending[env] : 0;
  const SgChain& C = H.chain[c];
  const double h = a.timestep;
  double* gq = a.qpos + (size_t)env * nv;
  double* gv = a.qvel + (size_t)env * nv;
  double* gw = a.warm + (size_t)env * nv;
  const double kenv = a.kenv[env];
  double q[SG_CD], v[SG_CD], w[SG_CD], kk[SG_CD], act = 0, ctrl = 0;
#pragma unroll
  for (int d = 0; d < SG_CD; d++) {
    int j = C.dof0 + d;
    if (a.do_reset) { q[d] = C.qpos0[d]; v[d] = 0; w[d] = 0; }
    else { q[d] = gq[j]; v[d] = gv[j]; w[d] = gw[j]; }
    kk[d] = a.kmask_jnt[j] ? kenv : C.stiffness[d];
  }
  if (C.has_act) {
    if (a.do_reset) a.ctrl[(size_t)env * nu + C.act_id] = 0;
    else { act = a.act[(size_t)env * nu + C.act_id]; ctrl = a.ctrl[(size_t)env * nu + C.act_id]; }
  }
  const double kten = C.has_ten ? (a.kmask_ten[C.ten_id] ? kenv : C.ten_k0) : 0.0;
  double* ch = W.chh + st * SG_CHW;
  bool bad_acc = false;
  if (status & (SG_FLAG_BADQPOS | SG_FLAG_BADQVEL | SG_FLAG_BADQACC)) return;

  SG_T(17);
  if (a.do_finish && pend) {
    double aF[SG_CD], qacc_c[SG_CD];
#pragma unroll
    for (int d = 0; d < SG_CD; d++) {
      aF[d] = W.saF[SG_SAF_INDEX(d, st, S)];
      qacc_c[d] = ch[SGH_QSM + d] + aF[d];
      if (isbad(qacc_c[d])) bad_acc = true;
    }
    ChainKin K;
    {
      double* kd = (double*)&K;
#pragma unroll
      for (int i = 0; i < SGH_N_K; i++) kd[i] = ch[SGH_K + i];
    }
    if (a.sens) {
      ChainMotion Mo;
      chain_motion(C, K, v, qacc_c, H.gravity, Mo);
      double* so = a.sens + (size_t)env * a.sens_stride;
      for (int s = 0; s < C.nsite; s++) {
        int bi = C.s_body[s];
        double r3[3], sm[9], t[3], t2[3], acc[3], out[3], sbp[3], sbm[9], bw[3], bal[3];
        chain_body_pose(K, bi, sbp, sbm);
        mulmat3(r3, sbm, C.s_pos[s]);
        mulmat33(sm, sbm, C.s_mat[s]);
        for (int k = 0; k < 3; k++) { bw[k] = bi == 0 ? Mo.w[0][k] : Mo.w[SG_CB - 1][k]; bal[k] = bi == 0 ? Mo.al[0][k] : Mo.al[SG_CB - 1][k]; }
        if (C.s_gyro_adr[s] >= 0) {
          mulmatT3(out, sm, bw);
          for (int k = 0; k < 3; k++) so[C.s_gyro_adr[s] + k] = out[k];
        }
        if (C.s_acc_adr[s] >= 0) {
          for (int k = 0; k < 3; k++) acc[k] = bi == 0 ? Mo.a[0][k] : Mo.a[SG_CB - 1][k];
          cross3(t, bal, r3); addscl3(acc, t, 1);
          cross3(t, bw, r3); cross3(t2, bw, t); addscl3(acc, t2, 1);
          mulmatT3(out, sm, acc);
          for (int k = 0; k < 3; k++) so[C.s_acc_adr[s] + k] = out[k];
        }
      }
    }
    if (bad_acc) {
      atomicOr(&W.status[env], SG_FLAG_BADQACC);
    } else {
#pragma unroll
      for (int d = 0; d < SG_CD; d++) w[d] = qacc_c[d];
      if (a.finish_integrate) {
        bool damp = false;
#pragma unroll
        for (int d = 0; d < SG_CD; d++) damp |= C.damping[d] > 0;
        double qa[SG_CD];
        if (damp) {
          double MhB[16], MhBinv[16], rhs[SG_CD], Mm[16];
#pragma unroll
          for (int i = 0; i < SGH_N_M; i++) { Mm[i] = ch[SGH_M + i]; MhB[i] = Mm[i]; }
#pragma unroll
          for (int d = 0; d < SG_CD; d++) MhB[5 * d] += h * C.damping[d];
          spd_inverse4(MhB, MhBinv);
#pragma unroll
          for (int a2 = 0; a2 < SG_CD; a2++) {
            double s2 = ch[SGH_QFRC + a2];
#pragma unroll
            for (int b2 = 0; b2 < SG_CD; b2++) s2 += Mm[4 * a2 + b2] * aF[b2];
            rhs[a2] = s2;
          }
#pragma unroll
          for (int a2 = 0; a2 < SG_CD; a2++) {
            double s2 = 0;
#pragma unroll
            for (int b2 = 0; b2 < SG_CD; b2++) s2 += MhBinv[4 * a2 + b2] * rhs[b2];
            qa[a2] = s2;
          }
        } else {
#pragma unroll
          for (int d = 0; d < SG_CD; d++) qa[d] = qacc_c[d];
        }
        act += h * ch[SGH_ACTDOT];
#pragma unroll
        for (int d = 0; d < SG_CD; d++) { v[d] += h * qa[d]; q[d] += h * v[d]; }
      }
    }
  }

  SG_T(18);
  if (a.do_begin && !bad_acc) {
    int bad = 0;
#pragma unroll
    for (int d = 0; d < SG_CD; d++) bad |= (isbad(q[d]) ? SG_FLAG_BADQPOS : 0) | (isbad(v[d]) ? SG_FLAG_BADQVEL : 0);
    if (bad) {
      atomicOr(&W.status[env], bad);
    } else {
      ChainKin K;
      ChainDyn D;
      chain_kinematics(C, q, K);
      SG_T(19);
      chain_dynamics(C, K, q, v, act, ctrl, kk, kten, H.gravity, D);
      SG_T(20);
      double rec[SG_CHW];
#pragma unroll
      for (int i = 0; i < SG_CHW; i++) rec[i] = 0.0;
#pragma unroll
      for (int d = 0; d < SG_CD; d++) { rec[SGH_QSM + d] = D.qacc_smooth[d]; rec[SGH_QFRC + d] = D.qfrc_smooth[d]; rec[SGH_V + d] = v[d]; rec[SGH_W + d] = w[d]; }
      rec[SGH_ACTDOT] = D.act_dot;
#pragma unroll
      for (int i = 0; i < SGH_N_M; i++) { rec[SGH_M + i] = D.M[i]; rec[SGH_MINV + i] = D.Minv[i]; W.sMinv[SG_MINV_INDEX(i, st, S)] = D.Minv[i]; }
      {
        const double* kd = (const double*)&K;
#pragma unroll
        for (int i = 0; i < SGH_N_K; i++) rec[SGH_K + i] = kd[i];
      }
#pragma unroll
      for (int g = 0; g < SG_CG; g++) {
        double t[3] = {0, 0, 0}, bp_[3] = {0, 0, 0}, bm_[9], bm2[9];
#pragma unroll
        for (int k = 0; k < 9; k++) bm2[k] = 0;
        if (g < C.ngeom) {
          chain_body_pose(K, C.g_body[g], bp_, bm_);
          mulmat3(t, bm_, C.g_pos[g]);
          mulmat33(bm2, bm_, C.g_mat[g]);
        }
#pragma unroll
        for (int k = 0; k < 3; k++) rec[SGH_BOX + SGH_N_BOX1 * g + k] = bp_[k] + t[k];
#pragma unroll
        for (int k = 0; k < 9; k++) rec[SGH_BOX + SGH_N_BOX1 * g + 3 + k] = bm2[k];
      }
      SG_T(21);
      LimitRows L;
      limits_build(C, q, v, D.qacc_smooth, w, L);
      rec[SGH_LIMACT] = (double)L.active;
#pragma unroll
      for (int k = 0; k < SG_MAXLIM; k++) { rec[SGH_LIMSIGN + k] = L.sign[k]; rec[SGH_LIMR + k] = L.R[k]; rec[SGH_LIMB + k] = L.b[k]; rec[SGH_LIMF + k] = L.f[k]; }
#pragma unroll
      for (int i = 0; i < (SGH_END + 1) / 2; i++) ((double2*)ch)[i] = make_double2(rec[2 * i], rec[2 * i + 1]);
    }
  }
  SG_T(22);
#pragma unroll
  for (int d = 0; d < SG_CD; d++) { int j = C.dof0 + d; gq[j] = q[d]; gv[j] = v[d]; gw[j] = w[d]; }
  if (C.has_act) a.act[(size_t)env * nu + C.act_id] = act;
  SG_T(23);
  SG_TEND();
}


hipError_t sg_launch_chain(const SgPhaseArgs& p, int nenv, hipStream_t s) {
  hipLaunchKernelGGL(sg_chain_kernel, dim3(2 * ((nenv + 63) / 64)), dim3(64), 0, s, p);
  return hipGetLastError();
}
hipError_t sg_launch_phase(const SgPhaseArgs& p, int rounds, bool nb, bool genpass, int nenv, hipStream_t s) {
#define SG_PHASE(r)                                                                                   \
  if (nb) {                                                                                           \
    hipLaunchKernelGGL((sg_phase_kernel<r, SG_X_CPL, true>), dim3(nenv), dim3(64), 0, s, p);                 \
    if (genpass && p.do_begin) hipLaunchKernelGGL((sg_phase_kernel<r, 2, true, true>), dim3(nenv < SG_GEN_GRID ? nenv : SG_GEN_GRID), dim3(64), 0, s, p); \
  } else {                                                                                            \
    hipLaunchKernelGGL((sg_phase_kernel<r, SG_X_CPL, false>), dim3(nenv), dim3(64), 0, s, p);                \
    if (genpass && p.do_begin) hipLaunchKernelGGL((sg_phase_kernel<r, 2, false, true>), dim3(nenv < SG_GEN_GRID ? nenv : SG_GEN_GRID), dim3(64), 0, s, p); \
  }
  switch (rounds) {
    case 1: SG_PHASE(1); break;
    case 2: SG_PHASE(2); break;
    case 3: SG_PHASE(3); break;
    default: SG_PHASE(4); break;
  }
#undef SG_PHASE
  return hipGetLastError();
}
```

### soft-grip_amd/csrc/sg_rows_host.h

```cpp
#pragma once
#include <string>
#include <vector>

#include "sg_plan.h"
#include "sg_work.h"

inline bool sg_rows_admits(const SgPlanHeader& H, std::string* err) {
  if (H.nnb > 0 && (H.nelem > SG_ROWS_MAX_NELEM || sizeof(double) * SG_ROWS_LDS_NB(4, H.nelem, H.eq_rounds, 1) > 160 * 1024)) {
    if (err) *err = "too many neighbour equality rows for the PGS kernel's LDS";
    return false;
  }
  return true;
}

struct SgRowsShape {
  int nelem = 0, eq_rounds = 0;
  int nb_mode = 0;
  bool two_words = false;
  int cst_rounds = 0;
  size_t tab_words = 0;
  size_t lds_doubles(int epw, int nsl) const {
    return nb_mode ? SG_ROWS_LDS_NB(epw, nelem, eq_rounds, nb_mode == 2) : SG_ROWS_LDS_FIX(epw, 8 * nsl);
  }
};
inline SgRowsShape sg_rows_shape(const SgPlanHeader& H) {
  SgRowsShape s;
  s.nelem = H.nelem; s.eq_rounds = H.eq_rounds;
  s.nb_mode = H.nnb > 0 ? SG_ROWS_NB_MODE(H.nelem, H.eq_rounds) : 0;
  s.two_words = s.nb_mode == 1;
  s.cst_rounds = s.nb_mode == 2 ? H.eq_rounds + 8 : 0;
  s.tab_words = s.nb_mode ? sizeof(double) / sizeof(unsigned) * SG_LDS_NB_ZERO((size_t)0, H.eq_rounds, s.nb_mode == 2) : 0;
  return s;
}

struct SgRowsTables {
  std::vector<SgEqSlot> sched;
  std::vector<unsigned> tab;
  std::vector<int> cpos;
};
inline void sg_rows_tables(const SgPlan& P, SgRowsTables* T) {
  const SgPlanHeader& H = P.h;
  T->sched = P.sched;
  SgEqSlot idle;
  idle.e = idle.p[0] = idle.p[1] = idle.p[2] = H.nelem;
  for (int g = 0; g < 8 * SG_EQ_SLOTS; g++) T->sched.push_back(idle);
  const std::vector<SgEqSlot>& sch = T->sched;
  const bool two_words = sg_rows_shape(H).two_words;
  T->tab.assign((two_words ? 4 : 2) * sch.size(), 0u);
  for (size_t i = 0; i < 2 * sch.size(); i++) {
    const SgEqSlot& sl = sch[i >> 1];
    const int h = (int)(i & 1);
    const unsigned x = h ? sl.p[1] : sl.e, y = h ? sl.p[2] : sl.p[0];
    if (two_words) { T->tab[2 * i] = sg_tab2_pack(x, y); T->tab[2 * i + 1] = sg_tab2_rec((unsigned)sl.e, (unsigned)h); }
    else T->tab[i] = sg_tab1_pack(x, y, (unsigned)sl.e, (unsigned)h);
  }
  T->cpos.assign(H.nelem, 0);
  for (size_t i = 0; i < P.sched.size(); i++)
    if (P.sched[i].e < H.nelem) T->cpos[P.sched[i].e] = (int)(i / SG_EQ_SLOTS) * 128 + 4 * (int)(i % SG_EQ_SLOTS);
}

template <class F>
bool sg_rows_work_each(SgWork& w, const SgPlanHeader& H, int rounds, size_t n, bool legacy, F&& f) {
  const size_t S = 2 * n, N = H.nelem;
  const bool slim = SG_PHASE_SLIM(rounds);
  return f(&w.crec, legacy ? SG_CAP * ((n + SG_EPW - 1) / SG_EPW + 1) * SG_RF * SG_SPW : 0) &&
         f(&w.ns, S) &&
         f(&w.crow, SG_ROW_INDEX(SG_CAP + 2, 0, 0, 0, (n + 7) / 8)) &&
         f(&w.cdummy, sg_row_dummy_index((n + 3) / 4, 0)) &&
         f(&w.envh, SG_ENVH_ROWS * n) &&
         f(&w.shared, n) && f(&w.pending, n) && f(&w.status, n) && f(&w.iters, n) && f(&w.ncon, n) && f(&w.nefc, n) && f(&w.touch, n) &&
         f(&w.sMinv, SGH_N_M * S) &&
         f(&w.saF, SG_CD * S) &&
         f(&w.lim_active, S) &&
         f(&w.lim, SGH_N_LIM * S) &&
         f(&w.as, n * N) && f(&w.eqf, n * N) && f(&w.eqb, n * N) && f(&w.eqR, n * N) && f(&w.asme, n * N) && f(&w.fsm, n * N) &&
         f(&w.chh, n * 2 * SG_CHW) &&
         f(&w.nbf, n * (3 * N + 1)) && f(&w.nbb, n * (3 * N + 1)) && f(&w.nbR, n * (3 * N + 1)) &&
         f(&w.cst, sg_rows_shape(H).cst_rounds ? SG_CST_INDEX((n + 3) / 4, 0, 0, H.eq_rounds + 8) : 0) &&
         f(&w.gcon, n * SG_GEN_MAXCON * SG_GEN_W) &&
         f(&w.gen, n) &&
         f(&w.gen_count, 4) &&
         f(&w.gen_list, n) &&
         f(&w.gpairs16, slim ? n * SG_PAIRS_CAP(4) : 0) &&
         f(&w.gcval, slim ? n * SG_MAXCH * 64 : 0);
}
```

### soft-grip_amd/csrc/sg_rows_layout.h

```cpp
#pragma once
#include <cstddef>
#include <hip/hip_runtime.h>

#include "sg_math.h"

#define SG_RK 16
enum SgRowField : int {
  SGR_JF0 = 0, SGR_JF1, SGR_JF2, SGR_JF3,
  SGR_JS = 4, SGR_B = 5,
  SGR_F = 6, SGR_AF = 7,
  SGR_A0 = 8, SGR_A1, SGR_A2,
  SGR_IMJS = 11,
  SGR_W0 = 12, SGR_W1, SGR_W2,
  SGR_R = 15,
};
enum SgQuadField : int {
  SGQ_P11 = 0, SGQ_P12, SGQ_P22,
  SGQ_SLIDER = 4,
  SGQ_E1 = 8, SGQ_E2, SGQ_COS, SGQ_SIN,
};
#define SG_ROW_PAIR(k) ((k) / 2)
#define SG_ROW_HALF(k) ((k) & 1)
__host__ __device__ constexpr int sg_row_pair(int field) { return SG_ROW_PAIR(field); }
__host__ __device__ constexpr int sg_row_half(int field) { return SG_ROW_HALF(field); }
#define SG_ROW_INDEX(slot, wave, k, lane, nwb) \
  ((((((size_t)(slot)) * ((nwb) + 2) + (wave)) * (SG_RK / 2) + SG_ROW_PAIR(k)) * 64 + (lane)) * 2 + SG_ROW_HALF(k))
constexpr int SG_ROW_BASE_PAIR = 4;
#define SG_ROW_IMM(k) ((SG_ROW_PAIR(k) - SG_ROW_BASE_PAIR) * 64)
__host__ __device__ constexpr int sg_row_imm(int field) { return SG_ROW_IMM(field); }
__host__ __device__ constexpr size_t sg_row_slot_stride(int nwb) { return (size_t)(nwb + 2) * (SG_RK / 2) * 64; }
__host__ __device__ constexpr size_t sg_row_dummy_index(size_t wave, int pair) { return (wave * (SG_RK / 2) + pair) * 128; }
static_assert(sg_row_pair(SGR_F) == sg_row_pair(SGR_AF) && sg_row_half(SGR_F) == 0, "f and A f are one pair: the solver's one 16-byte write-back");
static_assert(SG_RK % 2 == 0 && sg_row_pair(0) == 0 && sg_row_pair(SG_RK - 1) == SG_RK / 2 - 1 && SGR_R == SG_RK - 1, "16 fields, pairs 0 .. SG_RK / 2 - 1");
static_assert(sg_row_imm(0) * 16 >= -4096 && sg_row_imm(SG_RK - 1) * 16 <= 4095, "every pair within a global load's 13-bit signed immediate offset");

#define SG_NSL_LIST(X) X(8) X(14) X(20) X(26) X(29) X(32)
__host__ __device__ constexpr int sg_rows_nsl(int nelem) {
#define SG_NSL_HOLDS(v) if (v * 8 >= nelem) return v;
  SG_NSL_LIST(SG_NSL_HOLDS)
#undef SG_NSL_HOLDS
  return 32;
}

constexpr int SG_ROWS_LDS_SINK = 72;
#define SG_LDS_FIX_BR(AF, EPW, NR) ((AF) + (size_t)2 * (EPW) * (NR))
#define SG_LDS_FIX_RI(BR, EPW, NR) ((BR) + (size_t)2 * (EPW) * (NR))
#define SG_LDS_FIX_IC(RI, EPW, NR) ((RI) + (size_t)(EPW) * (NR))
#define SG_LDS_FIX_ZERO(IC, NR) ((IC) + (size_t)2 * (NR))
#define SG_LDS_FIX_END(ZERO) ((ZERO) + SG_ROWS_LDS_SINK)
#define SG_ROWS_NA_NB(N) (((N) + 2) & ~1)
#define SG_ROWS_GW_NB(N, CST) (((CST) ? 4 : 8) * ((N) + 1))
#define SG_LDS_NB_GS(AE, EPW, N) ((AE) + (size_t)(EPW) * SG_ROWS_NA_NB(N))
#define SG_LDS_NB_TAB(GS, EPW, N, CST) ((GS) + (size_t)(EPW) * SG_ROWS_GW_NB(N, CST))
#define SG_LDS_NB_ZERO(TAB, ROUNDS, CST) ((TAB) + (size_t)8 * ((CST) ? 1 : 2) * ((ROUNDS) + 8))
#define SG_LDS_NB_ENV(ZERO) ((ZERO) + SG_ROWS_LDS_SINK)
#define SG_LDS_NB_END(ENV, EPW) ((ENV) + (size_t)2 * (EPW))
#define SG_ROWS_LDS_FIX(EPW, NR) SG_LDS_FIX_END(SG_LDS_FIX_ZERO(SG_LDS_FIX_IC(SG_LDS_FIX_RI(SG_LDS_FIX_BR((size_t)0, EPW, NR), EPW, NR), EPW, NR), NR))
#define SG_ROWS_LDS_NB(EPW, N, ROUNDS, CST) SG_LDS_NB_END(SG_LDS_NB_ENV(SG_LDS_NB_ZERO(SG_LDS_NB_TAB(SG_LDS_NB_GS((size_t)0, EPW, N), EPW, N, CST), ROUNDS, CST)), EPW)
#define SG_ROWS_NB_MODE(N, ROUNDS) (sizeof(double) * SG_ROWS_LDS_NB(4, N, ROUNDS, 0) <= 40 * 1024 ? 1 : 2)

constexpr int SG_TAB1_YSH = 11, SG_TAB1_RSH = 22, SG_TAB2_YSH = 16;
__host__ __device__ constexpr unsigned sg_tab1_pack(unsigned sx, unsigned sy, unsigned e, unsigned h) { return (8u * sx) | ((8u * sy) << SG_TAB1_YSH) | ((2u * e + h) << SG_TAB1_RSH); }
__host__ __device__ constexpr unsigned sg_tab1_x(unsigned w) { return w & ((1u << SG_TAB1_YSH) - 1u); }
__host__ __device__ constexpr unsigned sg_tab1_y(unsigned w) { return (w >> SG_TAB1_YSH) & ((1u << (SG_TAB1_RSH - SG_TAB1_YSH)) - 1u); }
__host__ __device__ constexpr unsigned sg_tab1_rec(unsigned w) { return (w >> SG_TAB1_RSH) << 4; }
__host__ __device__ constexpr unsigned sg_tab2_pack(unsigned sx, unsigned sy) { return (8u * sx) | ((8u * sy) << SG_TAB2_YSH); }
__host__ __device__ constexpr unsigned sg_tab2_rec(unsigned e, unsigned h) { return 64u * e + 32u * h; }
__host__ __device__ constexpr unsigned sg_tab2_x(unsigned w) { return w & ((1u << SG_TAB2_YSH) - 1u); }
__host__ __device__ constexpr unsigned sg_tab2_y(unsigned w) { return w >> SG_TAB2_YSH; }
constexpr int SG_ROWS_MAX_NELEM = (1 << SG_TAB1_YSH) / 8 - 2;
static_assert(SG_ROWS_MAX_NELEM == 254 && 2 * SG_ROWS_MAX_NELEM + 1 < (1 << (32 - SG_TAB1_RSH)) && SG_TAB1_RSH - SG_TAB1_YSH >= SG_TAB1_YSH &&
              8 * (SG_ROWS_MAX_NELEM + 2) <= (1 << SG_TAB2_YSH), "every field of a table word holds its largest value");

#define SG_CST_INDEX(w, k, l, rounds) ((((size_t)(w) * (rounds) + (k)) * 64 + (l)) * 2)

__host__ __device__ constexpr size_t sg_eq_fix_index(size_t env, int e, int N) { return env * (size_t)N + (size_t)e; }
__host__ __device__ constexpr size_t sg_eq_nb_index(size_t env, int e, int d, int N) { return (env * (size_t)N + (size_t)e) * 3 + (size_t)d; }
__host__ __device__ constexpr int sg_eq_rec_trips(int nr) { return (4 * (nr + 1) + 63) / 64; }
__host__ __device__ constexpr int sg_eq_rec_row(int lane, int trip) { return lane + 64 * trip; }
__host__ __device__ constexpr bool sg_eq_rec_stored(int u, int N) { return u < 4 * (N + 1); }
__host__ __device__ constexpr bool sg_eq_rec_live(int u, int N) { return u < 4 * N; }
__host__ __device__ constexpr size_t sg_eq_rec_index(size_t env, int u, int N, size_t nenv) {
  const size_t envc = env < nenv ? env : nenv - 1;
  const int uc = u < 4 * N ? u : 4 * N - 1, e = uc >> 2, d = uc & 3;
  return d == 0 ? sg_eq_fix_index(envc, e, N) : sg_eq_nb_index(envc, e, d - 1, N);
}

#define SG_CHW 160
enum { SGH_QSM = 0, SGH_QFRC = 4, SGH_ACTDOT = 8, SGH_M = 9, SGH_K = 25, SGH_MINV = 73, SGH_V = 89, SGH_W = 93, SGH_BOX = 97,
       SGH_LIMACT = 121, SGH_LIMSIGN = 122, SGH_LIMR = 130, SGH_LIMB = 138, SGH_LIMF = 146, SGH_END = 154 };
constexpr int SGH_N_M = SG_CD * SG_CD;
constexpr int SGH_N_K = (int)(sizeof(sgm::ChainKin) / sizeof(double));
constexpr int SGH_N_BOX1 = 3 + 9, SGH_N_BOX = SGH_N_BOX1 * SG_CG;
constexpr int SGH_N_LIM = 4 * SG_MAXLIM;
struct SgHandoffField { int off, len; };
constexpr SgHandoffField SG_HANDOFF_FIELDS[] = {{SGH_QSM, SG_CD}, {SGH_QFRC, SG_CD}, {SGH_ACTDOT, 1}, {SGH_M, SGH_N_M}, {SGH_K, SGH_N_K}, {SGH_MINV, SGH_N_M},
                                                {SGH_V, SG_CD}, {SGH_W, SG_CD}, {SGH_BOX, SGH_N_BOX}, {SGH_LIMACT, 1}, {SGH_LIMSIGN, SG_MAXLIM},
                                                {SGH_LIMR, SG_MAXLIM}, {SGH_LIMB, SG_MAXLIM}, {SGH_LIMF, SG_MAXLIM}};
constexpr bool sg_handoff_tiles() {
  int at = 0;
  for (const SgHandoffField& f : SG_HANDOFF_FIELDS) {
    if (f.off != at || f.len <= 0) return false;
    at += f.len;
  }
  return at == SGH_END;
}
static_assert(SGH_N_K == 48 && sizeof(sgm::ChainKin) % sizeof(double) == 0, "ChainKin is 48 doubles: axes, anchors, body positions and rotations");
static_assert(sg_handoff_tiles() && SGH_END <= SG_CHW && SG_CHW % 2 == 0, "the hand-off fields tile [0, SGH_END) inside a record of 16-byte pairs");

enum SgEnvhRow : int { SG_ENVH_TB, SG_ENVH_TR, SG_ENVH_TA, SG_ENVH_TF, SG_ENVH_ROWS };
enum SgLimRow : int { SG_LIM_SIGN, SG_LIM_R, SG_LIM_B, SG_LIM_F, SG_LIM_ROWS };
static_assert(SGH_LIMSIGN + SG_LIM_R * SG_MAXLIM == SGH_LIMR && SGH_LIMSIGN + SG_LIM_B * SG_MAXLIM == SGH_LIMB && SGH_LIMSIGN + SG_LIM_F * SG_MAXLIM == SGH_LIMF &&
              SG_LIM_ROWS * SG_MAXLIM == SGH_N_LIM, "SgWork::lim is the hand-off record's limit block, value by value");
#define SG_STREAM(env, chain) (2 * (size_t)(env) + (chain))
#define SG_ENVH_INDEX(row, env, nenv) ((size_t)(row) * (nenv) + (env))
#define SG_MINV_INDEX(i, st, S) ((size_t)(i) * (S) + (st))
#define SG_SAF_INDEX(d, st, S) ((size_t)(d) * (S) + (st))
#define SG_LIM_INDEX(row, k, st, S) (((size_t)(row) * SG_MAXLIM + (k)) * (S) + (st))
#define SG_LIM_FLAT_INDEX(i, st, S) ((size_t)(i) * (S) + (st))
static_assert(SG_LIM_INDEX(SG_LIM_F, SG_MAXLIM - 1, 5, 7) == SG_LIM_FLAT_INDEX(SGH_N_LIM - 1, 5, 7), "the two views of SgWork::lim");
```

### soft-grip_amd/csrc/sg_work.h

```cpp
#pragma once
#include <hip/hip_runtime.h>

#include "../../include/softgrip.h"
#include "sg_math.h"
#include "sg_general.h"
#include "sg_rows_layout.h"

using namespace sgm;

#define SG_CAP 64
#define SG_NF 26
#define SG_RF 30
#define SG_REC_INDEX(slot, wave, field, pos, nwb) (((((size_t)(slot)) * ((nwb) + 1) + (wave)) * SG_RF + (field)) * SG_SPW + (pos))
#define SG_G 8
#define SG_EPW (64 / SG_G)
#define SG_SPW (2 * SG_EPW)
#define SG_GEN_GRID 256

struct SgWork {
  double* crec;
  unsigned long long* secprof;
  double* crow;
  double* cdummy;
  int* ns;
  double* envh;
  int *shared, *pending, *status, *iters, *ncon, *nefc, *touch;
  double *sMinv, *saF;
  int* lim_active;
  double* lim;
  double *as, *eqf, *eqb, *eqR;
  double *asme, *fsm;
  double* chh;
  double *nbf, *nbb, *nbR;
  double* cst;
  double* gcon;
  int* gen;
  int* gen_count;
  int* gen_list;
  unsigned short* gpairs16;
  double* gcval;
};

struct SgPhaseArgs {
  const SgPlanHeader* H;
  const double* elem;
  double *qpos, *qvel, *warm, *act, *ctrl;
  const double* kenv;
  const int *kmask_jnt, *kmask_ten;
  const unsigned char* mask;
  double* sens;
  long long sens_stride;
  SgWork w;
  int nenv;
  int do_reset, do_finish, finish_integrate, do_begin, first;
  int rowlayout;
  const int* nbtab;
  const int* cpos;
  int cst_rounds;
  const SgGenPair* gpairs;
  int nelem, nv, nu, elem_dof0, nchain, t0_id;
  double timestep;
};

__host__ __device__ constexpr int sg_rows_load_slot(int i, int ahead, int nsmax) { return i + ahead < nsmax ? i + ahead : -1; }

struct StageRec2 {
  double dist, pos[3], n[3];
  int sl, box;
};

struct ChainLds2 {
  double v[SG_CD], w[SG_CD], qacc_smooth[SG_CD], Minv[16];
  int lim_active, pad;
  double lim_sign[SG_MAXLIM], lim_R[SG_MAXLIM], lim_b[SG_MAXLIM], lim_f[SG_MAXLIM];
};
static_assert(offsetof(ChainLds2, lim_R) - offsetof(ChainLds2, lim_sign) == (SGH_LIMR - SGH_LIMSIGN) * sizeof(double) &&
              offsetof(ChainLds2, lim_b) - offsetof(ChainLds2, lim_sign) == (SGH_LIMB - SGH_LIMSIGN) * sizeof(double) &&
              offsetof(ChainLds2, lim_f) - offsetof(ChainLds2, lim_sign) == (SGH_LIMF - SGH_LIMSIGN) * sizeof(double), "ChainLds2's limit rows lie as the hand-off record's");

#define SG_PHASE_SLIM(R) ((R) >= 4)
#define SG_PAIRS_CAP(R) (SG_MAXCH * SG_CG * ((R) * 64 + 2))
template <int R, int CPL, bool NB>
struct Smem2 {
  ChainKin K[SG_MAXCH];
  ChainLds2 cs[SG_MAXCH];
  double boxp[SG_MAXCH * SG_CG][3], boxm[SG_MAXCH * SG_CG][9];
  double ve[R * 64], asme[R * 64], we[R * 64], as[R * 64];
  StageRec2 stage[SG_MAXCH][32 * CPL];
  unsigned short pairs[SG_PHASE_SLIM(R) ? 4 : SG_PAIRS_CAP(R)];
  unsigned char eslot[R * 64][SG_MAXCH * SG_CG];
  double cval[SG_PHASE_SLIM(R) ? 1 : SG_MAXCH * 32 * CPL];
};
#define SG_PAIR_CENTER 0xFFF

__device__ __forceinline__ double wave_sum2(double x) {
#pragma unroll
  for (int o = 32; o > 0; o >>= 1) x += __shfl_xor(x, o);
  return x;
}
__device__ __forceinline__ int lanes_below2(unsigned long long m) {
  return __builtin_amdgcn_mbcnt_hi((unsigned)(m >> 32), __builtin_amdgcn_mbcnt_lo((unsigned)m, 0));
}

#if defined(__HIP_DEVICE_COMPILE__)
#define SG_CONSTAS __attribute__((address_space(4)))
#else
#define SG_CONSTAS
#endif

#ifdef SG_SECTION_PROF
#define SG_T0() unsigned long long t_prev_ = __builtin_readcyclecounter(), t_acc_[26] = {0, 0, 0, 0, 0, 0, 0, 0, 0, 0, 0, 0, 0, 0, 0, 0, 0, 0, 0, 0, 0, 0, 0, 0, 0, 0}
#define SG_T(k)                                                   \
  do {                                                            \
    unsigned long long t_now_ = __builtin_readcyclecounter();     \
    t_acc_[k] += t_now_ - t_prev_;                                \
    t_prev_ = __builtin_readcyclecounter();                       \
  } while (0)
#define SG_TEND()                                                 \
  do {                                                            \
    if (threadIdx.x == 0)                                         \
      for (int k_ = 0; k_ < 26; k_++)                             \
        if (t_acc_[k_]) atomicAdd(&a.w.secprof[k_], t_acc_[k_]);  \
  } while (0)
#else
#define SG_T0()
#define SG_T(k)
#define SG_TEND()
#endif


struct SgPgsArgs {
  const unsigned* tab;
  const SgEqSlot* sched;
  const int* nbtab;
  const SgPlanHeader* H;
  const double* elem;
  SgWork w;
  int nenv;
};

hipError_t sg_launch_chain(const SgPhaseArgs& p, int nenv, hipStream_t s);
hipError_t sg_launch_phase(const SgPhaseArgs& p, int rounds, bool nb, bool genpass, int nenv, hipStream_t s);
hipError_t sg_rows_prepare();
hipError_t sg_launch_rows(const SgPgsArgs& a, int nsl, int nb , int epw, int nenv, size_t lds_bytes, hipStream_t s);
#ifdef SG_LEGACY_PIPELINES
struct SgKArgs;
hipError_t sg_legacy_prepare();
hipError_t sg_launch_pgs_split(const SgPgsArgs& a, int nenv, size_t lds_bytes, hipStream_t s);
hipError_t sg_launch_fused(const SgKArgs& a, int rounds, int nenv, hipStream_t s);
#endif
```

Before: 1.138 million env-steps/s.

## Precompute derived element constants, batch early loads, branchless box checks, LDS neighbour forces

Extends the per-element constant table with host-precomputed mass sums, inverse masses and summed neighbour inverse weights, so the phase kernel loads these instead of recomputing divisions. It also issues state, constant and chain hand-off loads unconditionally at clamped indices so they can be batched ahead of use, and stores displacement instead of position in LDS to skip repeated subtraction. It rewrites the box/box and plane overlap test as a branchless, ballot-gated lane computation. For small R it keeps a copy of the neighbour forces in LDS to avoid global reads. The extra registers and LDS may reduce occupancy.

```diff
diff --git a/soft-grip_amd/csrc/sg_api.hip b/soft-grip_amd/csrc/sg_api.hip
--- a/soft-grip_amd/csrc/sg_api.hip
+++ b/soft-grip_amd/csrc/sg_api.hip
@@ -72,7 +72,7 @@
   r.shape = sg_rows_shape(H);
   r.nsl = sg_rows_nsl(H.nelem);
   r.w.secprof = b->secprof;
-  bool ok = A.zeros(&r.H, 1) && hipMemcpy(r.H, &H, sizeof H, hipMemcpyHostToDevice) == hipSuccess && A.upload(&r.elem, m->plan.elem) &&
+  bool ok = A.zeros(&r.H, 1) && hipMemcpy(r.H, &H, sizeof H, hipMemcpyHostToDevice) == hipSuccess && A.upload(&r.elem, sg_rows_elem_table(m->plan)) &&
             A.upload(&r.gpairs, m->plan.gpairs) &&
             sg_rows_work_each(r.w, H, m->rounds, (size_t)b->n, SG_LEGACY_ON != 0, [&A](auto** p, size_t count) { return A.zeros(p, count); });
   if (ok && r.shape.nb_mode) {
diff --git a/soft-grip_amd/csrc/sg_phase.hip b/soft-grip_amd/csrc/sg_phase.hip
--- a/soft-grip_amd/csrc/sg_phase.hip
+++ b/soft-grip_amd/csrc/sg_phase.hip
@@ -9,13 +9,13 @@
   const double (*boxm)[9];
   const ChainKin* K;
   const ChainLds2* cs;
-  const double *qe, *ve, *asme, *we;
+  const double *dq, *ve, *asme, *we;
 };
 
 __device__ __forceinline__ void sg_gen_capsule(const SgPhaseArgs& a, const GenLds& L, int e, double* cp, double* cax) {
   const int N = a.nelem;
   auto EL = [&](int f, int k) { return a.elem[(size_t)f * N + k]; };
-  const double dq = L.qe[e] - EL(SGE_QPOS0, e);
+  const double dq = L.dq[e];
   cp[0] = EL(SGE_GX, e) + EL(SGE_AX, e) * dq; cp[1] = EL(SGE_GY, e) + EL(SGE_AY, e) * dq; cp[2] = EL(SGE_GZ, e) + EL(SGE_AZ, e) * dq;
   cax[0] = EL(SGE_CX, e); cax[1] = EL(SGE_CY, e); cax[2] = EL(SGE_CZ, e);
 }
@@ -235,7 +235,7 @@
   __shared__ Smem2<R, CPL, NB> Sm;
   const SG_CONSTAS double* const elemc = (const SG_CONSTAS double*)a.elem;
   [[maybe_unused]] const SG_CONSTAS int* const nbtabc = (const SG_CONSTAS int*)a.nbtab;
-  auto EL = [&](int f, int e) { return elemc[(size_t)f * N + e]; };
+  auto EL = [&](int f, int e) { return elemc[sg_elem_table_index(f, e, N)]; };
   const int half = lane >> 5;
   const bool high = half != 0;
   const bool is_chain_lane = (lane & 31) == 0 && half < nchain;
@@ -262,48 +262,77 @@
   const double kenv = a.kenv[env];
   const int kt0_masked = a.kmask_ten[a.t0_id];
 
-  double qe[R], ve[R], we[R], ke[R];
+  bool live[R];
+  int ec[R];
+#pragma unroll
+  for (int r = 0; r < R; r++) { const int e = r * 64 + lane; live[r] = e < N; ec[r] = live[r] ? e : N - 1; }
+  double qe[R], ve[R], we[R], ke[R], eq0[R];
+  {
+    double qs[R], vs[R], ws[R], k0[R];
+    int km[R];
+#pragma unroll
+    for (int r = 0; r < R; r++) {
+      qs[r] = gq[e0 + ec[r]]; vs[r] = gv[e0 + ec[r]]; ws[r] = gw[e0 + ec[r]];
+      km[r] = a.kmask_jnt[e0 + ec[r]]; k0[r] = EL(SGE_K0, ec[r]); eq0[r] = EL(SGE_QPOS0, ec[r]);
+    }
+#pragma unroll
+    for (int r = 0; r < R; r++) {
+      qe[r] = live[r] ? (a.do_reset ? eq0[r] : qs[r]) : 0.0;
+      ve[r] = live[r] && !a.do_reset ? vs[r] : 0.0;
+      we[r] = live[r] && !a.do_reset ? ws[r] : 0.0;
+      ke[r] = live[r] ? (km[r] ? kenv : k0[r]) : 0.0;
+    }
+  }
+  double ase[R], asme_p[R], fsm_p[R];
+  double msum[R], invm0[R], damp[R], coef[R];
 #pragma unroll
   for (int r = 0; r < R; r++) {
-    int e = r * 64 + lane;
-    qe[r] = ve[r] = we[r] = ke[r] = 0;
-    if (e < N) {
-      if (a.do_reset) { qe[r] = EL(SGE_QPOS0, e); }
-      else { qe[r] = gq[e0 + e]; ve[r] = gv[e0 + e]; we[r] = gw[e0 + e]; }
-      ke[r] = a.kmask_jnt[e0 + e] ? kenv : EL(SGE_K0, e);
-    }
-  }
-  double ase[R], asme_p[R], fsm_p[R];
-#pragma unroll
-  for (int r = 0; r < R; r++) {
-    const int e = r * 64 + lane;
-    ase[r] = asme_p[r] = fsm_p[r] = 0;
-    if (a.do_finish && e < N) {
-      ase[r] = W.as[(size_t)env * N + e]; asme_p[r] = W.asme[(size_t)env * N + e];
-      if (a.finish_integrate) fsm_p[r] = W.fsm[(size_t)env * N + e];
-    }
-  }
-  if (a.do_begin && half < nchain) {
-    const double* ch = W.chh + ((size_t)env * 2 + half) * SG_CHW;
-    double* const kd = (double*)&Sm.K[half];
-    double* const box = &Sm.boxp[half * SG_CG][0];
-    double* const boxm = &Sm.boxm[half * SG_CG][0];
-    double* const lim = CS.lim_sign;
-#pragma unroll
-    for (int j0 = 0; j0 < SG_CHW; j0 += 32) {
-      const int j = j0 + (lane & 31);
-      const double v = j < SG_CHW ? ch[j] : 0.0;
-      if (j >= SGH_QSM && j < SGH_QSM + SG_CD) CS.qacc_smooth[j - SGH_QSM] = v;
-      else if (j >= SGH_K && j < SGH_K + SGH_N_K) kd[j - SGH_K] = v;
-      else if (j >= SGH_MINV && j < SGH_MINV + SGH_N_M) CS.Minv[j - SGH_MINV] = v;
-      else if (j >= SGH_V && j < SGH_V + SG_CD) CS.v[j - SGH_V] = v;
-      else if (j >= SGH_W && j < SGH_W + SG_CD) CS.w[j - SGH_W] = v;
-      else if (j >= SGH_BOX && j < SGH_BOX + SGH_N_BOX) {
-        const int g = (j - SGH_BOX) / SGH_N_BOX1, k = (j - SGH_BOX) % SGH_N_BOX1;
-        if (k < 3) box[3 * g + k] = v; else boxm[9 * g + k - 3] = v;
-      }
-      else if (j == SGH_LIMACT) CS.lim_active = (int)v;
-      else if (j >= SGH_LIMSIGN && j < SGH_LIMSIGN + SGH_N_LIM) lim[j - SGH_LIMSIGN] = v;
+    const size_t o = (size_t)env * N + ec[r];
+    const double as_l = W.as[o], asme_l = W.asme[o], fsm_l = W.fsm[o];
+    const bool f = a.do_finish && live[r];
+    ase[r] = f ? as_l : 0.0; asme_p[r] = f ? asme_l : 0.0; fsm_p[r] = f && a.finish_integrate ? fsm_l : 0.0;
+    msum[r] = EL(SGD_MSUM, ec[r]); invm0[r] = EL(SGD_INVM, ec[r]); damp[r] = EL(SGE_DAMPING, ec[r]);
+    const double cf = EL(SGE_COEF, ec[r]);
+    coef[r] = live[r] ? cf : 0.0;
+  }
+  double eax[R][3], egp[R][3], emass[R], esref[R], eqlo[R], eqhi[R];
+  auto load_begin_consts = [&]() {
+#pragma unroll
+    for (int r = 0; r < R; r++) {
+      eax[r][0] = EL(SGE_AX, ec[r]); eax[r][1] = EL(SGE_AY, ec[r]); eax[r][2] = EL(SGE_AZ, ec[r]);
+      egp[r][0] = EL(SGE_GX, ec[r]); egp[r][1] = EL(SGE_GY, ec[r]); egp[r][2] = EL(SGE_GZ, ec[r]);
+      emass[r] = EL(SGE_MASS, ec[r]); esref[r] = EL(SGE_SPRINGREF, ec[r]); eqlo[r] = EL(SGE_QLO, ec[r]); eqhi[r] = EL(SGE_QHI, ec[r]);
+    }
+  };
+  constexpr bool CONSTS_EARLY = R <= 2;
+  if constexpr (CONSTS_EARLY) load_begin_consts();
+  {
+    const double* ch = W.chh + ((size_t)env * 2 + (half < nchain ? half : 0)) * SG_CHW;
+    static_assert(SG_CHW % 32 == 0, "whole trips of a half's 32 lanes");
+    double hv[SG_CHW / 32];
+#pragma unroll
+    for (int t = 0; t < SG_CHW / 32; t++) hv[t] = ch[32 * t + (lane & 31)];
+    if (a.do_begin && half < nchain) {
+      double* const kd = (double*)&Sm.K[half];
+      double* const box = &Sm.boxp[half * SG_CG][0];
+      double* const boxm = &Sm.boxm[half * SG_CG][0];
+      double* const lim = CS.lim_sign;
+#pragma unroll
+      for (int j0 = 0; j0 < SG_CHW; j0 += 32) {
+        const int j = j0 + (lane & 31);
+        const double v = hv[j0 / 32];
+        if (j >= SGH_QSM && j < SGH_QSM + SG_CD) CS.qacc_smooth[j - SGH_QSM] = v;
+        else if (j >= SGH_K && j < SGH_K + SGH_N_K) kd[j - SGH_K] = v;
+        else if (j >= SGH_MINV && j < SGH_MINV + SGH_N_M) CS.Minv[j - SGH_MINV] = v;
+        else if (j >= SGH_V && j < SGH_V + SG_CD) CS.v[j - SGH_V] = v;
+        else if (j >= SGH_W && j < SGH_W + SG_CD) CS.w[j - SGH_W] = v;
+        else if (j >= SGH_BOX && j < SGH_BOX + SGH_N_BOX) {
+          const int g = (j - SGH_BOX) / SGH_N_BOX1, k = (j - SGH_BOX) % SGH_N_BOX1;
+          if (k < 3) box[3 * g + k] = v; else boxm[9 * g + k - 3] = v;
+        }
+        else if (j == SGH_LIMACT) CS.lim_active = (int)v;
+        else if (j >= SGH_LIMSIGN && j < SGH_LIMSIGN + SGH_N_LIM) lim[j - SGH_LIMSIGN] = v;
+      }
     }
   }
   const bool dead = (status & (SG_FLAG_BADQPOS | SG_FLAG_BADQVEL | SG_FLAG_BADQACC)) != 0;
@@ -337,10 +366,10 @@
         we[r] = qacc_e[r];
         qa[r] = yc[r] = 0;
         if (e < N && a.finish_integrate) {
-          double m = EL(SGE_MASS, e) + EL(SGE_ARMATURE, e);
-          double den = m + h * EL(SGE_DAMPING, e);
+          double m = msum[r];
+          double den = m + h * damp[r];
           qa[r] = (fsm_p[r] + m * ase[r]) / den;
-          if (H.t0_implicit) { const double cf = EL(SGE_COEF, e); yc[r] = cf / den; Sp += cf * qa[r]; }
+          if (H.t0_implicit) { const double cf = coef[r]; yc[r] = cf / den; Sp += cf * qa[r]; }
         }
       }
       if (H.t0_implicit && a.finish_integrate) {
@@ -370,14 +399,11 @@
     if (__ballot(bad != 0)) {
       flags |= (__ballot(bad & 1) ? 1 : 0) | (__ballot(bad & 2) ? 2 : 0);
     } else {
-      double invm[R], asme[R], coef[R];
+      double invm[R], asme[R], dq[R];
       double L0p = 0, Ldp = 0;
-#pragma unroll
-      for (int r = 0; r < R; r++) {
-        int e = r * 64 + lane;
-        coef[r] = e < N ? EL(SGE_COEF, e) : 0.0;
-        L0p += coef[r] * qe[r]; Ldp += coef[r] * ve[r];
-      }
+      if constexpr (!CONSTS_EARLY) load_begin_consts();
+#pragma unroll
+      for (int r = 0; r < R; r++) { L0p += coef[r] * qe[r]; Ldp += coef[r] * ve[r]; }
       const double L0 = wave_sum2(L0p), Ld = wave_sum2(Ldp);
       const double frc_t0 = -kt0 * (L0 - H.t0_lspring) - H.t0_damping * Ld;
       int unsupported = 0, ns0 = 0, ns1 = 0, touch = 0;
@@ -387,21 +413,21 @@
 #pragma unroll
         for (int r = 0; r < R; r++) {
           int e = r * 64 + lane;
-          invm[r] = asme[r] = 0;
+          invm[r] = asme[r] = dq[r] = 0;
           cpos[r][0] = cpos[r][1] = cpos[r][2] = 1e30;
           if (e < N) {
-            double ax[3] = {EL(SGE_AX, e), EL(SGE_AY, e), EL(SGE_AZ, e)}, m = EL(SGE_MASS, e);
+            double ax[3] = {eax[r][0], eax[r][1], eax[r][2]}, m = emass[r];
             double bias = -m * dot3(H.gravity, ax);
-            double f = -ke[r] * (qe[r] - EL(SGE_SPRINGREF, e)) - EL(SGE_DAMPING, e) * ve[r] + coef[r] * frc_t0 - bias;
-            invm[r] = 1.0 / (m + EL(SGE_ARMATURE, e));
+            double f = -ke[r] * (qe[r] - esref[r]) - damp[r] * ve[r] + coef[r] * frc_t0 - bias;
+            invm[r] = invm0[r];
             asme[r] = f * invm[r];
             W.fsm[(size_t)env * N + e] = f; W.asme[(size_t)env * N + e] = asme[r];
-            double dq = qe[r] - EL(SGE_QPOS0, e);
-            cpos[r][0] = EL(SGE_GX, e) + ax[0] * dq; cpos[r][1] = EL(SGE_GY, e) + ax[1] * dq; cpos[r][2] = EL(SGE_GZ, e) + ax[2] * dq;
-            if (!(qe[r] > EL(SGE_QLO, e) && qe[r] < EL(SGE_QHI, e))) unsupported = 1;
+            dq[r] = qe[r] - eq0[r];
+            cpos[r][0] = egp[r][0] + ax[0] * dq[r]; cpos[r][1] = egp[r][1] + ax[1] * dq[r]; cpos[r][2] = egp[r][2] + ax[2] * dq[r];
+            if (!(qe[r] > eqlo[r] && qe[r] < eqhi[r])) unsupported = 1;
             Sm.ve[e] = ve[r]; Sm.asme[e] = asme[r]; Sm.we[e] = we[r];
             *(unsigned int*)&Sm.eslot[e][0] = 0u;
-            Sm.as[e] = qe[r];
+            Sm.as[e] = dq[r];
           }
         }
         SG_T(2);
@@ -466,7 +492,7 @@
             if (is_center) v0 = sphere_box(H.center_pos, H.center_radius, bp, bm, sz, H.con_margin, r0) && r0.dist < H.con_margin;
           }
           if (have && !is_center) {
-            const double dq = Sm.as[e] - EL(SGE_QPOS0, e);
+            const double dq = Sm.as[e];
             double cp[3] = {EL(SGE_GX, e) + EL(SGE_AX, e) * dq, EL(SGE_GY, e) + EL(SGE_AY, e) * dq, EL(SGE_GZ, e) + EL(SGE_AZ, e) * dq};
             double cax[3] = {EL(SGE_CX, e), EL(SGE_CY, e), EL(SGE_CZ, e)};
             int mk = capsule_box(cp, cax, H.cap_radius, H.cap_hl, bp, bm, sz, H.con_margin, r0, r1);
@@ -509,40 +535,42 @@
       }
       SG_T(3);
       {
-        int nb = nchain * SG_CG, npairs = nb * H.nstatic;
-        const double *p1 = nullptr, *R1 = nullptr, *s1 = nullptr, *p2 = nullptr, *R2 = nullptr, *s2 = nullptr;
-        double bd = 0;
-        bool pair = false;
-        if (lane < npairs) {
-          int b = lane / H.nstatic, s = lane % H.nstatic, c = b / SG_CG, g = b % SG_CG;
-          if (g < H.chain[c].ngeom) {
-            pair = true;
-            p1 = Sm.boxp[b]; R1 = Sm.boxm[b]; s1 = H.chain[c].g_size[g];
-            p2 = H.st_pos[s]; R2 = H.st_mat[s]; s2 = H.st_size[s];
-            bd = H.chain[c].g_rbound[g] + H.st_rbound[s];
-          }
-        } else if (lane >= 32 && lane < 32 + SG_CG * SG_CG && nchain == 2) {
-          int g = (lane - 32) / SG_CG, g2 = (lane - 32) % SG_CG;
-          if (g < H.chain[0].ngeom && g2 < H.chain[1].ngeom) {
-            int b = g, b2 = SG_CG + g2;
-            pair = true;
-            p1 = Sm.boxp[b]; R1 = Sm.boxm[b]; s1 = H.chain[0].g_size[g];
-            p2 = Sm.boxp[b2]; R2 = Sm.boxm[b2]; s2 = H.chain[1].g_size[g2];
-            bd = H.chain[0].g_rbound[g] + H.chain[1].g_rbound[g2];
-          }
-        }
-        if (pair) {
-          double dif[3] = {p1[0] - p2[0], p1[1] - p2[1], p1[2] - p2[2]};
-          if (dot3(dif, dif) <= bd * bd && box_box_overlap(p1, R1, s1, p2, R2, s2, 0)) unsupported = 1;
-        }
-        if (lane >= 48 && lane < 48 + SG_MAXCH * SG_CG && H.has_plane) {
-          int b = lane - 48, c = b / SG_CG, g = b % SG_CG;
-          if (c < nchain && g < H.chain[c].ngeom) {
-            double dif[3] = {Sm.boxp[b][0] - H.plane_pos[0], Sm.boxp[b][1] - H.plane_pos[1], Sm.boxp[b][2] - H.plane_pos[2]}, ext = 0;
-            for (int k = 0; k < 3; k++)
-              ext += H.chain[c].g_size[g][k] * fabs(H.plane_normal[0] * Sm.boxm[b][k] + H.plane_normal[1] * Sm.boxm[b][3 + k] + H.plane_normal[2] * Sm.boxm[b][6 + k]);
-            if (dot3(dif, H.plane_normal) - ext <= 0) unsupported = 1;
-          }
+        const int nb = nchain * SG_CG, nst = H.nstatic, npairs = nb * nst, nst1 = nst > 0 ? nst : 1;
+        const bool k_static = lane < npairs, k_boxes = !k_static && lane >= 32 && lane < 32 + SG_CG * SG_CG && nchain == 2;
+        const bool k_plane = lane >= 48 && lane < 48 + SG_MAXCH * SG_CG && H.has_plane;
+        static_assert(SG_MAXSTATIC * SG_MAXCH * SG_CG <= 48, "a plane lane has no pair");
+        const int b1 = k_static ? lane / nst1 : (k_boxes ? (lane - 32) / SG_CG : (k_plane ? lane - 48 : 0));
+        const int b2 = k_boxes ? SG_CG + (lane - 32) % SG_CG : 0, s = k_static ? lane % nst1 : 0;
+        const int c1 = b1 / SG_CG, g1 = b1 % SG_CG, c2 = b2 / SG_CG, g2 = b2 % SG_CG;
+        const SG_CONSTAS SgChain& C1 = H.chain[c1];
+        const SG_CONSTAS SgChain& C2 = H.chain[c2];
+        double p1[3], R1[9], s1[3], p2[3], R2[9], s2[3];
+        const int ng1 = C1.ngeom, ng2 = C2.ngeom;
+        const double rb1 = C1.g_rbound[g1], rb2 = k_boxes ? C2.g_rbound[g2] : H.st_rbound[s];
+#pragma unroll
+        for (int k = 0; k < 3; k++) {
+          p1[k] = Sm.boxp[b1][k]; s1[k] = C1.g_size[g1][k];
+          const double pb = Sm.boxp[b2][k], ps = H.st_pos[s][k], sb = C2.g_size[g2][k], ss = H.st_size[s][k];
+          p2[k] = k_boxes ? pb : ps; s2[k] = k_boxes ? sb : ss;
+        }
+#pragma unroll
+        for (int k = 0; k < 9; k++) {
+          R1[k] = Sm.boxm[b1][k];
+          const double mb = Sm.boxm[b2][k], ms = H.st_mat[s][k];
+          R2[k] = k_boxes ? mb : ms;
+        }
+        const bool pair = (k_static && g1 < ng1) || (k_boxes && g1 < ng1 && g2 < ng2);
+        const double bd = rb1 + rb2;
+        const double dif[3] = {p1[0] - p2[0], p1[1] - p2[1], p1[2] - p2[2]};
+        const bool near = pair && dot3(dif, dif) <= bd * bd;
+        if (__ballot(near)) {
+          if (near && box_box_overlap(p1, R1, s1, p2, R2, s2, 0)) unsupported = 1;
+        }
+        if (k_plane && c1 < nchain && g1 < ng1) {
+          double dp[3] = {p1[0] - H.plane_pos[0], p1[1] - H.plane_pos[1], p1[2] - H.plane_pos[2]}, ext = 0;
+          for (int k = 0; k < 3; k++)
+            ext += s1[k] * fabs(H.plane_normal[0] * R1[k] + H.plane_normal[1] * R1[3 + k] + H.plane_normal[2] * R1[6 + k]);
+          if (dot3(dp, H.plane_normal) - ext <= 0) unsupported = 1;
         }
         special = __ballot(unsupported) != 0;
       }
@@ -561,7 +589,7 @@
           GL.gas = (double*)&Sm.stage[0][0] + SG_GEN_MAXCON + SG_GEN_MAXCON / 2;
           GL.tmp = (double*)&Sm.stage[0][0] + 8 * SG_GEN_MAXCON; GL.gg = GL.tmp + 96;
           GL.boxp = Sm.boxp; GL.boxm = Sm.boxm; GL.K = Sm.K; GL.cs = Sm.cs;
-          GL.qe = Sm.as; GL.ve = Sm.ve; GL.asme = Sm.asme; GL.we = Sm.we;
+          GL.dq = Sm.as; GL.ve = Sm.ve; GL.asme = Sm.asme; GL.we = Sm.we;
           int gfl = 0, gtouch = 0;
           ngen = sg_gen_phase(a, *a.H, env, GL, &gfl, &gtouch);
           flags |= gfl;
@@ -611,7 +639,7 @@
           if (sl >= 0) {
             ax[0] = EL(SGE_AX, sl); ax[1] = EL(SGE_AY, sl); ax[2] = EL(SGE_AZ, sl);
             ve_ = Sm.ve[sl]; as_ = Sm.asme[sl]; we_ = Sm.we[sl];
-            im = 1.0 / (EL(SGE_MASS, sl) + EL(SGE_ARMATURE, sl)); bw = EL(SGE_BINVW, sl);
+            im = EL(SGD_INVM, sl); bw = EL(SGE_BINVW, sl);
           }
           contact_build(c, rec, Sm.K[half], nd, CS.Minv, CS.v, CS.qacc_smooth, CS.w, C.b_invw_tran[bi], sl, ax, ve_, as_, we_, im, bw, *a.H);
           csl_[k] = sl; cinvm[k] = c.invm;
@@ -709,13 +737,27 @@
       SG_T(5);
       double eqR[R], eqb[R], eqf[R];
       double tbp = 0, tjp = 0, tAp = 0;
+      double einvw[R];
+      [[maybe_unused]] int nbe2l[R][3], nbidl[R][3], nbin[R][3];
+      [[maybe_unused]] double nbw[R][3];
+#pragma unroll
+      for (int r = 0; r < R; r++) {
+        einvw[r] = EL(SGE_INVW, ec[r]);
+        if constexpr (NB) {
+#pragma unroll
+          for (int d = 0; d < 3; d++) {
+            nbe2l[r][d] = nbtabc[d * N + ec[r]]; nbidl[r][d] = nbtabc[(3 + d) * N + ec[r]]; nbin[r][d] = nbtabc[(6 + d) * N + ec[r]];
+            nbw[r][d] = EL(SGD_NBINVW + d, ec[r]);
+          }
+        }
+      }
 #pragma unroll
       for (int r = 0; r < R; r++) {
         int e = r * 64 + lane;
         eqR[r] = 1; eqb[r] = 0; eqf[r] = 0;
         if (e < N) {
-          double pos = qe[r] - EL(SGE_QPOS0, e), imp = impedance(H.eqj_solimp, pos, 0);
-          eqR[r] = fmax(SG_MINVAL, (1 - imp) / imp * EL(SGE_INVW, e));
+          double pos = dq[r], imp = impedance(H.eqj_solimp, pos, 0);
+          eqR[r] = fmax(SG_MINVAL, (1 - imp) / imp * einvw[r]);
           double aref = -H.eqj_B * ve[r] - H.eqj_K * imp * pos;
           eqb[r] = asme[r] - aref;
           eqf[r] = -(we[r] - aref) / eqR[r];
@@ -729,12 +771,14 @@
       [[maybe_unused]] double nbff[R][3];
       [[maybe_unused]] double nbbb[R][3];
       [[maybe_unused]] double* const gnbf = W.nbf + (size_t)env * 3 * N;
+      constexpr bool NBF_LDS = SG_PHASE_NBF_LDS(R, NB);
+      static_assert(!NBF_LDS || sizeof(Smem2<R, CPL, NB>) <= SG_PHASE_LDS_BUDGET, "the forces' LDS copy must leave eight workgroups per CU");
 #pragma unroll
       for (int r = 0; r < R; r++)
 #pragma unroll
         for (int d = 0; d < 3; d++) { nbe2[r][d] = -1; nbid[r][d] = -1; nbc0[r][d] = 0; nbff[r][d] = 0; nbbb[r][d] = 0; }
       if constexpr (NB) {
-        const double im0 = 1.0 / (EL(SGE_MASS, 0) + EL(SGE_ARMATURE, 0));
+        const double im0 = EL(SGD_INVM, 0);
         const SG_CONSTAS int* const cposc = (const SG_CONSTAS int*)a.cpos;
         const bool ready = a.rowlayout != 0, wantc = ready && a.cst_rounds;
 #pragma unroll
@@ -745,15 +789,16 @@
             if (ready) c4[0] = sg_div(im0, im0 + eqR[r]);
 #pragma unroll
             for (int d = 0; d < 3; d++) {
-              const int e2 = nbtabc[d * N + e];
+              const int e2 = nbe2l[r][d];
               if (e2 >= 0) {
-                const int id = nbtabc[(3 + d) * N + e];
-                const double pos = (qe[r] - EL(SGE_QPOS0, e)) - (Sm.as[e2] - EL(SGE_QPOS0, e2)), imp = impedance(H.eqj_solimp, pos, 0);
-                const double Rr = fmax(SG_MINVAL, (1 - imp) / imp * (EL(SGE_INVW, e) + EL(SGE_INVW, e2)));
+                const int id = nbidl[r][d];
+                const double pos = dq[r] - Sm.as[e2], imp = impedance(H.eqj_solimp, pos, 0);
+                const double Rr = fmax(SG_MINVAL, (1 - imp) / imp * nbw[r][d]);
                 const double aref = -H.eqj_B * (ve[r] - Sm.ve[e2]) - H.eqj_K * imp * pos;
                 const double bb = (asme[r] - Sm.asme[e2]) - aref, ff = -((we[r] - Sm.we[e2]) - aref) / Rr;
                 nbe2[r][d] = e2; nbid[r][d] = id; nbc0[r][d] = ff * (0.5 * Rr * ff + bb);
                 nbff[r][d] = ff; gnbf[id] = ff;
+                if constexpr (NBF_LDS) Sm.nbf[id] = ff;
                 nbbb[r][d] = bb;
                 if (ready) { g3[d] = fma(Rr, ff, bb); c4[1 + d] = sg_div(im0, 2.0 * im0 + Rr); }
                 else { W.nbb[(size_t)env * 3 * N + id] = bb; W.nbR[(size_t)env * 3 * N + id] = Rr; }
@@ -796,7 +841,11 @@
               for (int d = 0; d < 3; d++) if (nbid[r][d] >= 0) fe += nbff[r][d];
               double fin[3];
 #pragma unroll
-              for (int d = 0; d < 3; d++) { const int ii = nbtabc[(6 + d) * N + e]; fin[d] = ii >= 0 ? gnbf[ii] : 0.0; }
+              for (int d = 0; d < 3; d++) {
+                const int ii = nbin[r][d];
+                if constexpr (NBF_LDS) fin[d] = ii >= 0 ? Sm.nbf[ii] : 0.0;
+                else fin[d] = ii >= 0 ? gnbf[ii] : 0.0;
+              }
 #pragma unroll
               for (int d = 0; d < 3; d++) fe -= fin[d];
             }
@@ -900,6 +949,7 @@
             for (int d = 0; d < ND; d++)
               if (nbid[r][d] >= 0) {
                 nbff[r][d] = 0.0; gnbf[nbid[r][d]] = 0.0;
+                if constexpr (NBF_LDS) Sm.nbf[nbid[r][d]] = 0.0;
                 if (a.rowlayout) W.nbb[sg_eq_nb_index((size_t)env, r * 64 + lane, d, N)] = nbbb[r][d];
               }
           }
diff --git a/soft-grip_amd/csrc/sg_rows_host.h b/soft-grip_amd/csrc/sg_rows_host.h
--- a/soft-grip_amd/csrc/sg_rows_host.h
+++ b/soft-grip_amd/csrc/sg_rows_host.h
@@ -59,6 +59,24 @@
     if (P.sched[i].e < H.nelem) T->cpos[P.sched[i].e] = (int)(i / SG_EQ_SLOTS) * 128 + 4 * (int)(i % SG_EQ_SLOTS);
 }
 
+inline std::vector<double> sg_rows_elem_table(const SgPlan& P) {
+  const int N = P.h.nelem;
+  std::vector<double> t(P.elem);
+  t.resize(sg_elem_table_doubles(N), 0.0);
+  for (int e = 0; e < N; e++) {
+    const double m = t[sg_elem_table_index(SGE_MASS, e, N)], arm = t[sg_elem_table_index(SGE_ARMATURE, e, N)];
+    const double msum = m + arm;
+    t[sg_elem_table_index(SGD_MSUM, e, N)] = msum;
+    t[sg_elem_table_index(SGD_INVM, e, N)] = 1.0 / msum;
+    if (P.h.nnb > 0)
+      for (int d = 0; d < 3; d++) {
+        const int e2 = P.nbtab[(size_t)d * N + e];
+        if (e2 >= 0) t[sg_elem_table_index(SGD_NBINVW + d, e, N)] = t[sg_elem_table_index(SGE_INVW, e, N)] + t[sg_elem_table_index(SGE_INVW, e2, N)];
+      }
+  }
+  return t;
+}
+
 template <class F>
 bool sg_rows_work_each(SgWork& w, const SgPlanHeader& H, int rounds, size_t n, bool legacy, F&& f) {
   const size_t S = 2 * n, N = H.nelem;
diff --git a/soft-grip_amd/csrc/sg_rows_layout.h b/soft-grip_amd/csrc/sg_rows_layout.h
--- a/soft-grip_amd/csrc/sg_rows_layout.h
+++ b/soft-grip_amd/csrc/sg_rows_layout.h
@@ -86,6 +86,15 @@
   return d == 0 ? sg_eq_fix_index(envc, e, N) : sg_eq_nb_index(envc, e, d - 1, N);
 }
 
+enum SgElemDerived : int {
+  SGD_MSUM = SGE_NFIELD,
+  SGD_INVM,
+  SGD_NBINVW,
+  SGD_NFIELD = SGD_NBINVW + 3
+};
+__host__ __device__ constexpr size_t sg_elem_table_index(int f, int e, int N) { return (size_t)f * (size_t)N + (size_t)e; }
+__host__ __device__ constexpr size_t sg_elem_table_doubles(int N) { return (size_t)SGD_NFIELD * (size_t)N; }
+
 #define SG_CHW 160
 enum { SGH_QSM = 0, SGH_QFRC = 4, SGH_ACTDOT = 8, SGH_M = 9, SGH_K = 25, SGH_MINV = 73, SGH_V = 89, SGH_W = 93, SGH_BOX = 97,
        SGH_LIMACT = 121, SGH_LIMSIGN = 122, SGH_LIMR = 130, SGH_LIMB = 138, SGH_LIMF = 146, SGH_END = 154 };
diff --git a/soft-grip_amd/csrc/sg_work.h b/soft-grip_amd/csrc/sg_work.h
--- a/soft-grip_amd/csrc/sg_work.h
+++ b/soft-grip_amd/csrc/sg_work.h
@@ -80,6 +80,8 @@
 
 #define SG_PHASE_SLIM(R) ((R) >= 4)
 #define SG_PAIRS_CAP(R) (SG_MAXCH * SG_CG * ((R) * 64 + 2))
+#define SG_PHASE_LDS_BUDGET (160 * 1024 / 8)
+#define SG_PHASE_NBF_LDS(R, NB) ((NB) && (R) <= 2)
 template <int R, int CPL, bool NB>
 struct Smem2 {
   ChainKin K[SG_MAXCH];
@@ -90,6 +92,7 @@
   unsigned short pairs[SG_PHASE_SLIM(R) ? 4 : SG_PAIRS_CAP(R)];
   unsigned char eslot[R * 64][SG_MAXCH * SG_CG];
   double cval[SG_PHASE_SLIM(R) ? 1 : SG_MAXCH * 32 * CPL];
+  double nbf[SG_PHASE_NBF_LDS(R, NB) ? 3 * R * 64 : 1];
 };
 #define SG_PAIR_CENTER 0xFFF
 
```

Measured after the change: 1.163 million env-steps/s, median of 6. +2.2%, better.
